# VITA-Group/MM3DGS-SLAM

Measured on AMD Instinct MI355X. Metric: SLAM frames/sec (track+map), TUM fr1/desk-shaped 640x480, higher is better.
Workload: dtype f32

## Files before the change

mm3dgs_slam_amd/csrc/api.hip:

```cpp
#include <math.h>
#include <stdarg.h>
#include <stdio.h>
#include <string.h>
#include "mm3dgs_common.h"
#include <algorithm>
#include "fused_api.h"

static thread_local char g_err[512] = "";
static int fail(int code, const char* fmt, ...) {
  va_list ap;
  va_start(ap, fmt);
  vsnprintf(g_err, sizeof(g_err), fmt, ap);
  va_end(ap);
  return code;
}
static int check_launch(const char* what) {
  hipError_t e = hipGetLastError();
  if (e != hipSuccess) return fail(-10, "%s: %s", what, hipGetErrorString(e));
  return 0;
}

#include <mutex>
#include <vector>
struct KernelProfile {
  std::vector<std::pair<hipEvent_t, hipEvent_t>> pending, pool;
  unsigned long long launches = 0;
  double total_ms = 0.0;
};
static KernelProfile g_prof[MM3DGS_PROF_KERNELS];
static std::mutex g_prof_mu;
static int g_prof_on = 0;
struct ProfScope {
  int k; hipStream_t s; hipEvent_t e1 = nullptr; bool on;
  ProfScope(int k_, hipStream_t s_) : k(k_), s(s_), on(g_prof_on == 1 || (g_prof_on == 2 && (k_ == MM3DGS_PROF_COMPOSITE_BWD || k_ == MM3DGS_PROF_COMPOSITE_BWD_TRACK ||
                                                                                     k_ == MM3DGS_PROF_COMPOSITE_FWD || k_ == MM3DGS_PROF_TRACK_FWD_BWD))) {
    if (on && g_prof_on == 2) {
      static unsigned long long sample[MM3DGS_PROF_KERNELS] = {};
      on = (sample[k_]++ & 63ull) == 0ull;
    }
    if (!on) return;
    std::lock_guard<std::mutex> lk(g_prof_mu);
    std::pair<hipEvent_t, hipEvent_t> ev;
    if (!g_prof[k].pool.empty()) { ev = g_prof[k].pool.back(); g_prof[k].pool.pop_back(); }
    else { (void)hipEventCreate(&ev.first); (void)hipEventCreate(&ev.second); }
    g_prof[k].pending.push_back(ev);
    e1 = ev.second;
    (void)hipEventRecord(ev.first, s);
  }
  ~ProfScope() { if (on) (void)hipEventRecord(e1, s); }
};

__global__ void profile_null_kernel() {}

extern "C" {

void mm3dgs_profile_enable(int on) { g_prof_on = on; }
double mm3dgs_profile_event_overhead_ms(void* stream) {
  hipStream_t s = (hipStream_t)stream;
  hipEvent_t a, b;
  if (hipEventCreate(&a) != hipSuccess || hipEventCreate(&b) != hipSuccess) return 0.0;
  double t[2] = {0.0, 0.0};
  const int reps = 32;
  for (int n = 1; n <= 2; n++) {
    for (int r = 0; r < reps + 4; r++) {
      (void)hipEventRecord(a, s);
      for (int q = 0; q < n; q++) hipLaunchKernelGGL(profile_null_kernel, dim3(1), dim3(64), 0, s);
      (void)hipEventRecord(b, s);
      (void)hipEventSynchronize(b);
      float ms = 0.f;
      if (r >= 4 && hipEventElapsedTime(&ms, a, b) == hipSuccess) t[n - 1] += ms;
    }
  }
  (void)hipEventDestroy(a); (void)hipEventDestroy(b);
  const double o = (2.0 * t[0] - t[1]) / reps;
  return o > 0.0 ? o : 0.0;
}
int mm3dgs_profile_read(int kernel, uint64_t* launches, double* total_ms) {
  if (kernel < 0 || kernel >= MM3DGS_PROF_KERNELS) return fail(-1, "bad kernel id %d", kernel);
  std::lock_guard<std::mutex> lk(g_prof_mu);
  KernelProfile& p = g_prof[kernel];
  for (auto& ev : p.pending) {
    if (hipEventSynchronize(ev.second) == hipSuccess) {
      float ms = 0.f;
      if (hipEventElapsedTime(&ms, ev.first, ev.second) == hipSuccess) { p.total_ms += ms; p.launches++; }
    }
    p.pool.push_back(ev);
  }
  p.pending.clear();
  if (launches) *launches = p.launches;
  if (total_ms) *total_ms = p.total_ms;
  p.launches = 0; p.total_ms = 0.0;
  return 0;
}

const char* mm3dgs_last_error(void) { return g_err; }
int mm3dgs_version(void) { return MM3DGS_ABI_VERSION; }

size_t mm3dgs_geom_bytes(int P) { return geom_bytes_impl(P > 0 ? P : 1); }
size_t mm3dgs_image_bytes(int H, int W) { return image_bytes_impl(H, W); }
size_t mm3dgs_binning_bytes(size_t N) { return binning_bytes_impl(N); }
size_t mm3dgs_backward_scratch_bytes(int P, size_t N) { return bwd_bytes_impl(P, N); }

static int check_common(const Mm3dgsCamera* cam, int P, int M, int C, const float* shs, const float* colors,
                        const float* scales, const float* rots, const float* cov3d) {
  if (!cam) return fail(-1, "camera is NULL");
  if (cam->image_height <= 0 || cam->image_width <= 0) return fail(-1, "bad image size %dx%d", cam->image_height, cam->image_width);
  if (cam->image_height > 16 * 65535 || cam->image_width > 16 * 65535) return fail(-1, "image too large for 16-bit tile coordinates");
  if (P < 0) return fail(-1, "P < 0");
  if (C < 1 || C > MM3DGS_MAX_CHANNELS) return fail(-1, "C=%d outside 1..%d", C, MM3DGS_MAX_CHANNELS);
  if (P == 0) return 0;
  if (!shs && !colors) return fail(-2, "Please provide excatly one of either SHs or precomputed colors!");
  if (shs) {
    if (C < 3) return fail(-2, "SH colour needs C >= 3");
    if (C > 3 && !colors) return fail(-2, "C=%d with SHs needs %d extra precomputed channels", C, C - 3);
    if (cam->sh_degree < 0 || cam->sh_degree > 3) return fail(-2, "sh_degree %d outside 0..3", cam->sh_degree);
    if (M < (cam->sh_degree + 1) * (cam->sh_degree + 1)) return fail(-2, "M=%d too small for sh_degree %d", M, cam->sh_degree);
  }
  if ((scales == nullptr || rots == nullptr) == (cov3d == nullptr))
    return fail(-2, "Please provide exactly one of either scale/rotation pair or precomputed 3D covariance!");
  if (!cam->bg || !cam->viewmatrix || !cam->projmatrix || !cam->campos) return fail(-1, "camera device pointers missing");
  return 0;
}

int mm3dgs_forward_geom(const Mm3dgsCamera* cam, int P, int M, int C, const float* means3D, const float* shs,
                        const float* colors_precomp, const float* opacities, const float* scales,
                        const float* rotations, const float* cov3D_precomp, int32_t* radii, void* geom_state,
                        void* image_state, uint32_t* host_num_rendered, void* stream) {
  int rc = check_common(cam, P, M, C, shs, colors_precomp, scales, rotations, cov3D_precomp);
  if (rc) return rc;
  if (!geom_state || !image_state || (P > 0 && (!means3D || !opacities || !radii))) return fail(-1, "NULL buffer");
  hipStream_t s = (hipStream_t)stream;
  CamDev cd = cam_dev(cam);
  GeomView g = geom_view(geom_state, P > 0 ? P : 1);
  ImageView iv = image_view(image_state, cd.H, cd.W);
  if (hipMemsetAsync(image_state, 0, iv.zero_bytes, s) != hipSuccess) return fail(-10, "memset failed");
  { ProfScope ps(MM3DGS_PROF_PREPROCESS_FWD, s);
    launch_preprocess_fwd(cd, P, M, C, means3D, shs, colors_precomp, opacities, scales, rotations, cov3D_precomp, radii, g, iv, s); }
  { ProfScope ps(MM3DGS_PROF_SCAN, s); launch_scan_tiles(cd.gx * cd.gy, P, g, iv, s); }
  if (host_num_rendered)
    if (hipMemcpyAsync(host_num_rendered, &iv.hdr->num_rendered, sizeof(uint32_t), hipMemcpyDeviceToHost, s) != hipSuccess)
      return fail(-10, "num_rendered copy failed");
  return check_launch("forward_geom");
}

int mm3dgs_forward_raster(const Mm3dgsCamera* cam, int P, int C, const void* geom_state, void* image_state,
                          void* binning_state, size_t N_capacity, float* out_color, void* stream) {
  if (!cam || !geom_state || !image_state || !binning_state || !out_color) return fail(-1, "NULL buffer");
  if (C < 1 || C > MM3DGS_MAX_CHANNELS) return fail(-1, "C=%d outside 1..%d", C, MM3DGS_MAX_CHANNELS);
  hipStream_t s = (hipStream_t)stream;
  CamDev cd = cam_dev(cam);
  GeomView g = geom_view((void*)geom_state, P > 0 ? P : 1);
  ImageView iv = image_view(image_state, cd.H, cd.W);
  BinView b = bin_view(binning_state, N_capacity);
  { ProfScope ps(MM3DGS_PROF_BIN_SORT, s); launch_scatter_sort(cd, P, g, iv, b, N_capacity, nullptr, s); }
  { ProfScope ps(MM3DGS_PROF_COMPOSITE_FWD, s); launch_composite_fwd(cd, C, g, iv, b, N_capacity, out_color, s); }
  return check_launch("forward_raster");
}

int mm3dgs_forward(const Mm3dgsCamera* cam, int P, int M, int C, const float* means3D, const float* shs,
                   const float* colors_precomp, const float* opacities, const float* scales,
                   const float* rotations, const float* cov3D_precomp, float* out_color, int32_t* radii,
                   void* geom_state, void* image_state, void* binning_state, size_t N_capacity, void* stream) {
  int rc = mm3dgs_forward_geom(cam, P, M, C, means3D, shs, colors_precomp, opacities, scales, rotations, cov3D_precomp,
                               radii, geom_state, image_state, nullptr, stream);
  if (rc) return rc;
  return mm3dgs_forward_raster(cam, P, C, geom_state, image_state, binning_state, N_capacity, out_color, stream);
}

int mm3dgs_backward(const Mm3dgsCamera* cam, int P, int M, int C, const float* means3D, const float* shs,
                    const float* colors_precomp, const float* opacities, const float* scales,
                    const float* rotations, const float* cov3D_precomp, const int32_t* radii,
                    const void* geom_state, const void* image_state, const void* binning_state,
                    size_t N_capacity, const float* dL_dout, void* backward_scratch, float* dL_dmeans3D,
                    float* dL_dmeans2D, float* dL_dshs, float* dL_dcolors_precomp, float* dL_dopacities,
                    float* dL_dscales, float* dL_drotations, float* dL_dcov3D, float* dL_dview, float* dL_dproj,
                    float* dL_dcampos, int flags, void* stream) {
  int rc = check_common(cam, P, M, C, shs, colors_precomp, scales, rotations, cov3D_precomp);
  if (rc) return rc;
  if (!geom_state || !image_state || !binning_state || !dL_dout || !backward_scratch || (P > 0 && !radii))
    return fail(-1, "NULL buffer");
  hipStream_t s = (hipStream_t)stream;
  CamDev cd = cam_dev(cam);
  GeomView g = geom_view((void*)geom_state, P > 0 ? P : 1);
  ImageView iv = image_view((void*)image_state, cd.H, cd.W);
  BinView b = bin_view((void*)binning_state, N_capacity);
  BwdView bw = bwd_view(backward_scratch, P, N_capacity);
  { ProfScope ps(MM3DGS_PROF_COMPOSITE_BWD, s); launch_composite_bwd(cd, C, g, iv, b, N_capacity, dL_dout, bw.dsub, s); }
  ProfScope ps_pb(MM3DGS_PROF_PREPROCESS_BWD, s);
  bool want_cam = dL_dview || dL_dproj || dL_dcampos;
  launch_preprocess_bwd(cd, P, M, C, means3D, shs, colors_precomp, opacities, scales, rotations, cov3D_precomp, radii, g, b,
                        N_capacity, bw, dL_dmeans3D, dL_dmeans2D, dL_dshs, dL_dcolors_precomp, dL_dopacities, dL_dscales, dL_drotations,
                        dL_dcov3D, want_cam, flags, s);
  if (want_cam) launch_camgrad_finish(bw, dL_dview, dL_dproj, dL_dcampos, s);
  return check_launch("backward");
}

static void warn_env_once() {
  static const bool done = [] {
    static const char* const names[] = {"MM3DGS_NO_DIRECT_BINS", "MM3DGS_NO_FUSED_SORT", "MM3DGS_NO_FUSED_SCAN", "MM3DGS_NO_FUSED_TRACK", "MM3DGS_NO_FOLDED_LOSS",
                                        "MM3DGS_NO_FORWARD_ROWS", "MM3DGS_NO_FUSED_PROJECT", "MM3DGS_NO_TILE_ORDER", "MM3DGS_NO_POSE_CHAIN", "MM3DGS_TILEMAP",
                                        "MM3DGS_DIRECT_MAX_TILES", "MM3DGS_STATS", "MM3DGS_SLAM_LDS_PAD", "MM3DGS_FWD_LDS_PAD", "MM3DGS_BWD_LDS_PAD"};
    for (const char* n : names) {
      const char* v = getenv(n);
      if (v && *v) fprintf(stderr, "mm3dgs: developer switch %s=%s is set in the environment: it changes which kernels run (include/mm3dgs.h, \"Environment\")\n", n, v);
    }
    return true;
  }();
  (void)done;
}

static SlamIn slam_in(const Mm3dgsSlamInputs* in) {
  SlamIn s;
  s.pose = in->pose; s.xyz = in->xyz; s.f_dc = in->f_dc; s.opacity = in->opacity; s.scaling = in->scaling;
  s.rotation = in->rotation; s.isotropic = in->isotropic; s.world = in->world_means;
  s.sh_deg = (in->f_rest && in->sh_degree > 0) ? in->sh_degree : 0;
  s.f_rest = s.sh_deg ? in->f_rest : nullptr; s.n_rest = s.sh_deg ? in->n_rest : 0;
  s.sh_dir = s.sh_deg ? in->sh_dir : 0;
  return s;
}
static int check_slam(const Mm3dgsCamera* cam, int P, const Mm3dgsSlamInputs* in) {
  warn_env_once();
  if (!cam || !in) return fail(-1, "NULL argument");
  if (cam->image_height <= 0 || cam->image_width <= 0) return fail(-1, "bad image size");
  if (P < 0) return fail(-1, "P < 0");
  if (!cam->bg || !cam->projmatrix) return fail(-1, "camera device pointers missing");
  if (!in->pose) return fail(-1, "pose is NULL");
  if (P > 0 && (!in->xyz || !in->f_dc || !in->opacity || !in->scaling || !in->rotation)) return fail(-1, "NULL Gaussian parameter");
  if (in->sh_degree < 0 || in->sh_degree > 3) return fail(-2, "sh_degree %d outside 0..3", in->sh_degree);
  if (in->sh_dir < 0 || in->sh_dir > 2) return fail(-2, "sh_dir %d outside 0..2", in->sh_dir);
  if (in->sh_degree > 0) {
    if (P > 0 && !in->f_rest) return fail(-2, "sh_degree %d needs the f_rest rows", in->sh_degree);
    if (in->n_rest < (in->sh_degree + 1) * (in->sh_degree + 1) - 1 || in->n_rest > 15) return fail(-2, "n_rest = %d does not hold sh_degree %d (or exceeds 15)", in->n_rest, in->sh_degree);
    if (in->world_means && in->sh_dir != 2) return fail(-2, "world_means = 1 needs sh_dir = 2 (direction from the camera centre), got sh_dir = %d", in->sh_dir);
    if (in->sh_dir == 2 && !in->world_means) return fail(-2, "sh_dir = 2 (direction from the camera centre) needs world_means = 1");
  }
  return 0;
}

static bool slam_fused_sort(int flags) {
  static const int no_fused_sort = env_flag("MM3DGS_NO_FUSED_SORT", 0);
  return (flags & MM3DGS_FWD_SHORT_LISTS) && !no_fused_sort;
}

struct DirectBins { bool on; uint32_t bin_cap, rec_cap, trec_cap; int nblocks, slot_bits; };
static DirectBins slam_direct_bins(int flags, const CamDev& cd, int P, size_t N_capacity) {
  static const int no_direct = env_flag("MM3DGS_NO_DIRECT_BINS", 0);
  static const int no_fused_scan = env_flag("MM3DGS_NO_FUSED_SCAN", 0);
  static const int max_tiles = env_flag("MM3DGS_DIRECT_MAX_TILES", 11264);
  DirectBins d;
  const int T = cd.gx * cd.gy;
  d.nblocks = (P + 255) / 256;
  const size_t nb = (size_t)std::max(d.nblocks, 1);
  d.slot_bits = direct_slot_bits(P);
  d.bin_cap = (uint32_t)std::min<size_t>(N_capacity / (size_t)std::max(T, 1), (size_t)((1u << std::max(d.slot_bits, 1)) - 1u));
  d.rec_cap = (uint32_t)std::min<size_t>((size_t)NLIST * N_capacity / nb, 0xffffffffull / nb);
  d.trec_cap = (uint32_t)std::min<size_t>(N_capacity / nb, 0xffffffffull / nb);
  d.on = (flags & MM3DGS_FWD_DIRECT_BINS) && (flags & MM3DGS_FWD_STATE_CLEAN) && slam_fused_sort(flags) && !no_direct && !no_fused_scan &&
         P > 0 && d.slot_bits >= DIRECT_SLOT_BITS_MIN && T <= max_tiles && T <= MAX_LDS_TILES && d.bin_cap >= 32 && d.rec_cap >= 1024 && d.trec_cap >= 256 &&
         N_capacity >= 4 * (size_t)P;
  return d;
}

static bool slam_tile_table(int flags) { return (flags & MM3DGS_FWD_STATE_CLEAN) && !env_flag("MM3DGS_NO_TILE_ORDER", 0); }
static void slam_refresh_tile_order(const Mm3dgsCamera* cam, void* image_state, int flags, void* stream) {
  if (!cam || !image_state || !slam_tile_table(flags) || cam->image_height <= 0 || cam->image_width <= 0) return;
  if (flags & MM3DGS_FWD_KEEP_TILE_ORDER) return;
  const CamDev cd = cam_dev(cam);
  launch_tile_order(cd.gx * cd.gy, cd.H, cd.W, image_view(image_state, cd.H, cd.W), (hipStream_t)stream);
}

static int slam_forward_impl(const Mm3dgsCamera* cam, int P, const Mm3dgsSlamInputs* in, float* out_color, int32_t* radii,
                             void* geom_state, void* image_state, void* binning_state, size_t N_capacity, int flags, void* stream,
                             const TrackLoss* tl, float* track_dsub = nullptr, bool projected = false, bool pose_chain = false) {
  int rc = check_slam(cam, P, in);
  if (rc) return rc;
  if (!out_color || !geom_state || !image_state || !binning_state || (P > 0 && !radii)) return fail(-1, "NULL buffer");
  hipStream_t s = (hipStream_t)stream;
  CamDev cd = cam_dev(cam);
  GeomView g = geom_view(geom_state, P > 0 ? P : 1);
  ImageView iv = image_view(image_state, cd.H, cd.W);
  BinView b = bin_view(binning_state, N_capacity);
  if (!(flags & MM3DGS_FWD_STATE_CLEAN))
    if (hipMemsetAsync(image_state, 0, iv.zero_bytes, s) != hipSuccess) return fail(-10, "memset failed");
  cd.sort_single = (flags & MM3DGS_FWD_SHORT_LISTS) ? 1 : 0;
  cd.bg_extras = 1;
  cd.state_clean = (flags & MM3DGS_FWD_STATE_CLEAN) ? 1 : 0;
  cd.tile_table = slam_tile_table(flags) ? 1 : 0;
  cd.fused_scan = ((flags & MM3DGS_FWD_STATE_CLEAN) && P > 0 && cd.gx * cd.gy <= MAX_FUSED_SCAN_TILES && !env_flag("MM3DGS_NO_FUSED_SCAN", 0)) ? 1 : 0;
  const bool fused_sort = slam_fused_sort(flags);
  if (tl && !fused_sort) return fail(-1, "internal: folded tracking loss needs the fused sort path");
  const DirectBins db = slam_direct_bins(flags, cd, P, N_capacity);
  cd.trec_cap = db.on ? db.trec_cap : 0u;
  if (db.on) {
    if (!projected) { ProfScope ps(MM3DGS_PROF_PREPROCESS_FWD, s); launch_slam_project_bin(cd, P, slam_in(in), radii, g, iv, b, db.bin_cap, db.rec_cap, db.slot_bits, s, pose_chain); }
    { ProfScope ps(track_dsub ? MM3DGS_PROF_TRACK_FWD_BWD : MM3DGS_PROF_COMPOSITE_FWD, s);
      if (track_dsub) launch_sort_composite_fwd_bwd_track(cd, g, iv, b, N_capacity, out_color, 1, s, *tl, db.nblocks, track_dsub, db.bin_cap, db.slot_bits, pose_chain);
      else launch_sort_composite_fwd6(cd, g, iv, b, N_capacity, out_color, 1, s, tl, db.nblocks, db.bin_cap, db.slot_bits); }
    return check_launch("slam_forward");
  }
  { ProfScope ps(MM3DGS_PROF_PREPROCESS_FWD, s); launch_slam_preprocess_fwd(cd, P, slam_in(in), radii, g, iv, s, nullptr, false, pose_chain); }
  if (!cd.fused_scan) { ProfScope ps(MM3DGS_PROF_SCAN, s); launch_scan_tiles(cd.gx * cd.gy, P, g, iv, s, (flags & MM3DGS_FWD_STATE_CLEAN) ? 1 : 0); }
  { ProfScope ps(MM3DGS_PROF_BIN_SORT, s); launch_scatter_sort(cd, P, g, iv, b, N_capacity, nullptr, s, fused_sort); }
  { ProfScope ps((fused_sort && track_dsub) ? MM3DGS_PROF_TRACK_FWD_BWD : MM3DGS_PROF_COMPOSITE_FWD, s);
    if (fused_sort && track_dsub) launch_sort_composite_fwd_bwd_track(cd, g, iv, b, N_capacity, out_color, (cd.fused_scan || cd.state_clean) ? 1 : 0, s, *tl, 0, track_dsub, 0, DIRECT_SLOT_BITS_MAX, pose_chain);
    else if (fused_sort) launch_sort_composite_fwd6(cd, g, iv, b, N_capacity, out_color, (cd.fused_scan || cd.state_clean) ? 1 : 0, s, tl);
    else launch_composite_fwd(cd, 6, g, iv, b, N_capacity, out_color, s); }
  return check_launch("slam_forward");
}

int mm3dgs_slam_visibility(const Mm3dgsCamera* cam, int P, const Mm3dgsSlamInputs* in, int32_t* radii, uint32_t* seen_count, void* geom_state,
                           void* stream) {
  int rc = check_slam(cam, P, in);
  if (rc) return rc;
  if (!geom_state || (P > 0 && !radii)) return fail(-1, "NULL buffer");
  CamDev cd = cam_dev(cam);
  GeomView g = geom_view(geom_state, P > 0 ? P : 1);
  ImageView iv = {};
  launch_slam_preprocess_fwd(cd, P, slam_in(in), radii, g, iv, (hipStream_t)stream, seen_count, true);
  return check_launch("slam_visibility");
}

int mm3dgs_slam_forward(const Mm3dgsCamera* cam, int P, const Mm3dgsSlamInputs* in, float* out_color, int32_t* radii,
                        void* geom_state, void* image_state, void* binning_state, size_t N_capacity, int flags, void* stream) {
  return slam_forward_impl(cam, P, in, out_color, radii, geom_state, image_state, binning_state, N_capacity, flags, stream, nullptr, nullptr,
                           (flags & MM3DGS_FWD_PROJECTED) != 0);
}

static int map_adam_dev(const Mm3dgsMapAdam* map_adam, MapAdam& ma) {
  if (map_adam->step < 1) return fail(-1, "map Adam step must be >= 1");
  for (int i = 0; i < 5; i++) {
    if (!map_adam->param[i] || !map_adam->exp_avg[i] || !map_adam->exp_avg_sq[i]) return fail(-2, "map Adam group %d has a NULL pointer", i);
    ma.p[i] = map_adam->param[i]; ma.m[i] = map_adam->exp_avg[i]; ma.v[i] = map_adam->exp_avg_sq[i];
    ma.step_size[i] = (float)(map_adam->lr[i] / (1.0 - pow(map_adam->beta1, (double)map_adam->step)));
  }
  ma.omb1 = (float)(1.0 - map_adam->beta1); ma.beta2 = (float)map_adam->beta2; ma.omb2 = (float)(1.0 - map_adam->beta2);
  ma.eps = (float)map_adam->eps;
  ma.bc2s = (float)sqrt(1.0 - pow(map_adam->beta2, (double)map_adam->step));
  ma.opt_mask = map_adam->opt_mask;
  ma.rp = map_adam->rest_param; ma.rm = map_adam->rest_exp_avg; ma.rv = map_adam->rest_exp_avg_sq;
  if (ma.rp && (!ma.rm || !ma.rv)) return fail(-2, "map Adam: the f_rest group has a NULL moment pointer");
  ma.rest_step_size = (float)(map_adam->rest_lr / (1.0 - pow(map_adam->beta1, (double)map_adam->step)));
  ma.on = 1;
  return 0;
}

static int slam_backward_impl(const Mm3dgsCamera* cam, int P, const Mm3dgsSlamInputs* in, const int32_t* radii,
                              const void* geom_state, const void* image_state, const void* binning_state, size_t N_capacity,
                              const float* dL_dout, void* backward_scratch, const Mm3dgsSlamGrads* grads, float* dL_dpose,
                              const Mm3dgsPoseAdam* pose_adam, const Mm3dgsMapAdam* map_adam, int flags, void* stream, const TrackLoss* tl,
                              float* prior_loss4 = nullptr, int dl_planes = 6, bool compositor_done = false, const float* fuse_next_pose = nullptr,
                              bool* fused_out = nullptr, bool pose_chain = false) {
  PoseLossScale pls = {nullptr, 0, 0.f, nullptr};
  if (tl && tl->defer_scale) { pls.rows = tl->partial; pls.nrows = ((tl->cfg.W + 15) / 16) * ((tl->cfg.H + 15) / 16); pls.w_l1 = tl->cfg.w_l1; pls.loss4 = tl->loss4; }
  int rc = check_slam(cam, P, in);
  if (rc) return rc;
  if (!geom_state || !image_state || !binning_state || !dL_dout || !backward_scratch || (P > 0 && !radii)) return fail(-1, "NULL buffer");
  hipStream_t s = (hipStream_t)stream;
  CamDev cd = cam_dev(cam);
  GeomView g = geom_view((void*)geom_state, P > 0 ? P : 1);
  ImageView iv = image_view((void*)image_state, cd.H, cd.W);
  BinView b = bin_view((void*)binning_state, N_capacity);
  BwdView bw = bwd_view(backward_scratch, P, N_capacity);
  cd.bg_extras = 1;
  cd.tile_table = slam_tile_table(flags) ? 1 : 0;
  const DirectBins db_bwd = slam_direct_bins(flags, cd, P, N_capacity);
  cd.trec_cap = db_bwd.on ? db_bwd.trec_cap : 0u;
  SlamGrads sg = {};
  if (grads) {
    const bool any = grads->d_xyz || grads->d_f_dc || grads->d_opacity || grads->d_scaling || grads->d_rotation;
    const bool all = grads->d_xyz && grads->d_f_dc && grads->d_opacity && grads->d_scaling && grads->d_rotation;
    if (any && !all) return fail(-2, "Gaussian gradient outputs must be all set or all NULL");
    if (grads->max_radii2D && (!grads->grad_accum || !grads->denom)) return fail(-2, "statistics outputs must be all set or all NULL");
    sg.d_xyz = grads->d_xyz; sg.d_f_dc = grads->d_f_dc; sg.d_opacity = grads->d_opacity; sg.d_scaling = grads->d_scaling;
    sg.d_rotation = grads->d_rotation; sg.max_radii2D = grads->max_radii2D; sg.grad_accum = grads->grad_accum; sg.denom = grads->denom;
    sg.d_f_rest = (all && in->sh_degree > 0) ? grads->d_f_rest : nullptr;
    if (all && in->sh_degree > 0 && !grads->d_f_rest) return fail(-2, "sh_degree > 0: the gradient outputs need d_f_rest too");
  }
  PoseAdam pa = {};
  if (pose_adam && pose_adam->pose) {
    if (!pose_adam->m || !pose_adam->v || !pose_adam->step) return fail(-2, "pose Adam state missing");
    pa.pose = pose_adam->pose; pa.m = pose_adam->m; pa.v = pose_adam->v; pa.step = pose_adam->step;
    pa.lr_q = pose_adam->lr_q; pa.lr_t = pose_adam->lr_t; pa.beta1 = pose_adam->beta1; pa.beta2 = pose_adam->beta2; pa.eps = (float)pose_adam->eps;
    if (pose_adam->prior_pose && (pose_adam->prior_w_t != 0.f || pose_adam->prior_w_q != 0.f)) {
      pa.prior = pose_adam->prior_pose; pa.prior_w_t = pose_adam->prior_w_t; pa.prior_w_q = pose_adam->prior_w_q;
    }
    pa.best = pose_adam->best;
  }
  MapAdam ma;
  memset(&ma, 0, sizeof(ma));
  if (map_adam)
    if (int rc2 = map_adam_dev(map_adam, ma)) return rc2;
  const bool sh = in->sh_degree > 0 && in->f_rest;
  if (sh && ma.on && !ma.rp) return fail(-2, "sh_degree > 0: the map Adam state needs the f_rest group");
  const bool tracking = sg.d_xyz == nullptr && !ma.on && !sh;
  if (tl && !tracking && !tl->dmaps) return fail(-1, "internal: a loss folded into the mapping backward needs the SSIM maps");
  if (pose_chain && !tracking) return fail(-1, "internal: the pose chain is a tracking-mode path");
  if (!compositor_done)
  { ProfScope ps(tracking ? MM3DGS_PROF_COMPOSITE_BWD_TRACK : MM3DGS_PROF_COMPOSITE_BWD, s);
    launch_composite_bwd_slam(cd, tracking, g, iv, b, N_capacity, dL_dout, bw.dsub, s, tl, dl_planes, pose_chain); }
  if (pose_chain) {
    ProfScope ps(MM3DGS_PROF_PREPROCESS_BWD, s);
    launch_slam_pose_finish(bw.dsub, cd.gx * cd.gy, in->pose, dL_dpose, pa, s, pls.rows ? &pls : nullptr, prior_loss4, &iv.hdr->overflow);
    return check_launch("slam_backward");
  }
  const bool fuse = fuse_next_pose && !tracking && ma.on && db_bwd.on && !dL_dpose && !pa.pose && !sg.d_xyz && !sh;
  if (fused_out) *fused_out = fuse;
  if (fuse) {
    ProfScope ps(MM3DGS_PROF_PREPROCESS_BWD, s);
    launch_slam_bwd_project(cd, P, slam_in(in), (int32_t*)radii, g, image_view((void*)image_state, cd.H, cd.W), b, N_capacity, bw, sg, ma, fuse_next_pose,
                            db_bwd.bin_cap, db_bwd.rec_cap, db_bwd.slot_bits, s);
  } else
  { ProfScope ps(MM3DGS_PROF_PREPROCESS_BWD, s); launch_slam_preprocess_bwd(cd, P, slam_in(in), radii, g, b, N_capacity, bw, sg, dL_dpose, pa, ma, s, pls.rows ? &pls : nullptr, prior_loss4, db_bwd.on, &iv.hdr->overflow); }
  return check_launch("slam_backward");
}

int mm3dgs_slam_backward(const Mm3dgsCamera* cam, int P, const Mm3dgsSlamInputs* in, const int32_t* radii,
                         const void* geom_state, const void* image_state, const void* binning_state, size_t N_capacity,
                         const float* dL_dout, void* backward_scratch, const Mm3dgsSlamGrads* grads, float* dL_dpose,
                         const Mm3dgsPoseAdam* pose_adam, const Mm3dgsMapAdam* map_adam, int flags, void* stream) {
  return slam_backward_impl(cam, P, in, radii, geom_state, image_state, binning_state, N_capacity, dL_dout, backward_scratch, grads, dL_dpose,
                            pose_adam, map_adam, flags, stream, nullptr);
}

static size_t loss_rows(int H, int W) { return (size_t)((W + 15) / 16) * ((H + 15) / 16); }
static LossCfg loss_cfg_dev(const Mm3dgsLossConfig* c) {
  LossCfg lc;
  lc.H = c->H; lc.W = c->W; lc.w_l1 = c->w_l1; lc.w_ssim = c->w_ssim; lc.w_pearson = c->w_pearson; lc.l1_mask = c->l1_mask;
  lc.pearson_mask = c->pearson_mask; lc.pearson_invert = c->pearson_invert; lc.sil_thr = c->sil_thr;
  for (int i = 0; i < 11; i++) lc.window[i] = c->window[i];
  lc.w_depth = c->w_depth_l1; lc.depth_mask = c->depth_l1_mask; lc.l1_sum = c->l1_sum;
  return lc;
}
static bool loss_is_variant(const Mm3dgsLossConfig* c) { return c->w_depth_l1 != 0.f || c->l1_sum != 0 || (c->l1_mask & 2) != 0; }
static int loss_cfg_check(const Mm3dgsLossConfig* c, const float* ref) {
  if (c->w_pearson != 0.f && !ref) return fail(-2, "Pearson term needs a reference depth");
  if ((c->w_depth_l1 != 0.f || (c->l1_mask & 2)) && !ref) return fail(-2, "depth-L1 term / { ref > 0 } mask needs a reference depth");
  if (c->w_depth_l1 != 0.f && c->w_pearson != 0.f) return fail(-2, "the depth-L1 and Pearson terms are exclusive");
  return 0;
}
size_t mm3dgs_loss_work_bytes(int H, int W) {
  return 256 + align_up((size_t)9 * H * W * 4, 256) + align_up(loss_rows(H, W) * 12 * 8, 256);
}

int mm3dgs_loss(const Mm3dgsLossConfig* c, const float* out6, const float* gt_color, const float* ref, void* work, float* dL,
                float* loss4, void* stream) {
  if (!c || !out6 || !gt_color || !work || !dL) return fail(-1, "NULL argument");
  if (c->H <= 0 || c->W <= 0) return fail(-1, "bad image size");
  if ((double)c->H * c->W * 36.0 >= 4294967296.0) return fail(-1, "image too large for the loss kernels' 32-bit offsets");
  if (int rc = loss_cfg_check(c, ref)) return rc;
  LossCfg lc = loss_cfg_dev(c);
  hipStream_t s = (hipStream_t)stream;
  ProfScope ps(MM3DGS_PROF_LOSS, s);
  char* w = (char*)work;
  launch_loss(lc, out6, gt_color, ref, (float*)(w + 256), (double*)w, (double*)(w + 256 + align_up((size_t)9 * c->H * c->W * 4, 256)), dL,
              loss4, s);
  return check_launch("loss");
}

int mm3dgs_slam_track(int n_iter, const Mm3dgsCamera* cam, int P, const Mm3dgsSlamInputs* in, float* out_color, int32_t* radii,
                      void* geom_state, void* image_state, void* binning_state, size_t N_capacity, int fwd_flags,
                      const Mm3dgsLossConfig* loss_cfg, const float* gt_color, const float* ref, void* loss_work, float* dL_dout,
                      float* loss4, void* backward_scratch, const Mm3dgsPoseAdam* pose_adam, void* stream) {
  if (n_iter < 0) return fail(-1, "n_iter < 0");
  if (!pose_adam || !pose_adam->pose) return fail(-2, "tracking needs the pose Adam state");
  Mm3dgsSlamGrads none;
  memset(&none, 0, sizeof(none));
  if (!loss_cfg || !gt_color || !loss_work || !dL_dout) return fail(-1, "NULL argument");
  if (int rc = loss_cfg_check(loss_cfg, ref)) return rc;
  const int no_fold = env_flag("MM3DGS_NO_FOLDED_LOSS", 0);
  const bool sh = in->sh_degree > 0 && in->f_rest;
  const bool fold = !no_fold && !sh && !loss_is_variant(loss_cfg) && loss_cfg->w_ssim == 0.f && slam_fused_sort(fwd_flags) && cam->image_height > 0 && cam->image_width > 0;
  TrackLoss tl = {};
  if (fold) {
    tl.cfg = loss_cfg_dev(loss_cfg);
    char* w = (char*)loss_work;
    tl.gt = gt_color; tl.ref = ref; tl.out = out_color; tl.sums = (const double*)w;
    tl.partial = (double*)(w + 256 + align_up((size_t)9 * loss_cfg->H * loss_cfg->W * 4, 256));
    tl.loss4 = loss4;
    tl.defer_scale = loss_cfg->w_pearson == 0.f ? 1 : 0;
    if (loss_cfg->H != cam->image_height || loss_cfg->W != cam->image_width) return fail(-1, "loss and camera image sizes differ");
  }
  const bool fuse_track = fold && tl.defer_scale && !env_flag("MM3DGS_NO_FUSED_TRACK", 0) && backward_scratch;
  float* track_dsub = nullptr;
  if (fuse_track) {
    track_dsub = bwd_view(backward_scratch, P, N_capacity).dsub;
  }
  const bool pose_chain = !in->world_means && !sh && backward_scratch && !env_flag("MM3DGS_NO_POSE_CHAIN", 0) &&
                          bwd_bytes_impl(P, N_capacity) >= (size_t)tiles_x(cam->image_width) * tiles_y(cam->image_height) * 32 * sizeof(float);
  if (n_iter > 0) slam_refresh_tile_order(cam, image_state, fwd_flags, stream);
  for (int it = 0; it < n_iter; it++) {
    int rc = slam_forward_impl(cam, P, in, out_color, radii, geom_state, image_state, binning_state, N_capacity, fwd_flags, stream, fold ? &tl : nullptr, track_dsub, false, pose_chain);
    if (rc) return rc;
    if (fold) {
      if (!tl.defer_scale) {
        ProfScope ps(MM3DGS_PROF_LOSS, (hipStream_t)stream);
        launch_loss_finish(tl.cfg, (double*)loss_work, tl.partial, (hipStream_t)stream);
      }
    } else {
      rc = mm3dgs_loss(loss_cfg, out_color, gt_color, ref, loss_work, dL_dout, loss4, stream);
      if (rc) return rc;
    }
    rc = slam_backward_impl(cam, P, in, radii, geom_state, image_state, binning_state, N_capacity, dL_dout, backward_scratch, &none,
                            nullptr, pose_adam, nullptr, fwd_flags, stream, fold ? &tl : nullptr, loss4, 6, fuse_track, nullptr, nullptr, pose_chain);
    if (rc) return rc;
  }
  return 0;
}

int mm3dgs_slam_map(int n_iter, const Mm3dgsMapView* views, const Mm3dgsCamera* cam, int P, const Mm3dgsSlamInputs* in, float* out_color,
                    int32_t* radii, void* geom_state, void* image_state, void* binning_state, size_t N_capacity, int fwd_flags,
                    const Mm3dgsLossConfig* loss_cfg, void* loss_work, float* dL_dout, float* loss4, void* backward_scratch,
                    const Mm3dgsSlamGrads* grads_stats, const Mm3dgsMapAdam* map_adam, void* stream) {
  if (n_iter < 0) return fail(-1, "n_iter < 0");
  if (n_iter > 0 && (!views || !in)) return fail(-1, "NULL argument");
  if (n_iter > 0 && !map_adam && !(grads_stats && grads_stats->d_xyz)) return fail(-1, "neither an Adam state nor gradient outputs");
  Mm3dgsSlamGrads sg;
  memset(&sg, 0, sizeof(sg));
  if (grads_stats) sg = *grads_stats;
  Mm3dgsMapAdam ad;
  memset(&ad, 0, sizeof(ad));
  if (map_adam) ad = *map_adam;
  Mm3dgsSlamInputs si = *in;
  if (n_iter > 0 && (!loss_cfg || !loss_work || !dL_dout)) return fail(-1, "NULL argument");
  const int no_rows = env_flag("MM3DGS_NO_FORWARD_ROWS", 0);
  const bool rows = n_iter > 0 && !no_rows && !loss_is_variant(loss_cfg) && loss_cfg->w_ssim != 0.f && slam_fused_sort(fwd_flags) && loss_cfg->H == cam->image_height &&
                    loss_cfg->W == cam->image_width;
  TrackLoss tl = {};
  LossCfg lc = {};
  char* w = (char*)loss_work;
  double* sums = (double*)w;
  float* dmaps = (float*)(w + 256);
  double* partial = n_iter > 0 ? (double*)(w + 256 + align_up((size_t)9 * loss_cfg->H * loss_cfg->W * 4, 256)) : nullptr;
  if (rows) {
    lc = loss_cfg_dev(loss_cfg);
    tl.cfg = lc; tl.out = out_color; tl.sums = sums; tl.partial = partial; tl.loss4 = nullptr; tl.defer_scale = 0;
  }
  const int no_fuse_proj = env_flag("MM3DGS_NO_FUSED_PROJECT", 0);
  bool projected = (fwd_flags & MM3DGS_FWD_PROJECTED) != 0;
  if (n_iter > 0) slam_refresh_tile_order(cam, image_state, fwd_flags, stream);
  for (int it = 0; it < n_iter; it++) {
    if (!views[it].pose || !views[it].gt_color) return fail(-1, "view %d: NULL pose or colour target", it);
    if (loss_cfg->w_pearson != 0.f && !views[it].ref_depth_or_null) return fail(-2, "view %d: Pearson term needs a reference depth", it);
    if ((loss_cfg->w_depth_l1 != 0.f || (loss_cfg->l1_mask & 2)) && !views[it].ref_depth_or_null) return fail(-2, "view %d: depth-L1 term needs a reference depth", it);
    si.pose = views[it].pose;
    int rc;
    if (rows) {
      tl.gt = views[it].gt_color; tl.ref = views[it].ref_depth_or_null;
      rc = slam_forward_impl(cam, P, &si, out_color, radii, geom_state, image_state, binning_state, N_capacity, fwd_flags, stream, &tl, nullptr, projected);
      if (rc) return rc;
      const bool fold_grad = !env_flag("MM3DGS_NO_FOLDED_LOSS", 0);
      { ProfScope ps(MM3DGS_PROF_LOSS, (hipStream_t)stream);
        launch_loss_after_forward_rows(lc, out_color, tl.gt, tl.ref, dmaps, sums, partial, fold_grad ? nullptr : dL_dout, (hipStream_t)stream); }
      if (loss4 && it == n_iter - 1) launch_loss_finish(lc, sums, partial, (hipStream_t)stream, loss4);
      rc = check_launch("loss");
      if (rc) return rc;
      tl.dmaps = fold_grad ? dmaps : nullptr;
      if (views[it].pose_adam_or_null && views[it].dpose_out_or_null) return fail(-2, "view %d: either a pose step or a pose-gradient output", it);
      const float* next_pose = (!no_fuse_proj && map_adam && it + 1 < n_iter && !views[it].pose_adam_or_null && !views[it + 1].pose_adam_or_null &&
                                !views[it].dpose_out_or_null && views[it + 1].pose) ? views[it + 1].pose : nullptr;
      projected = false;
      rc = slam_backward_impl(cam, P, &si, radii, geom_state, image_state, binning_state, N_capacity, dL_dout, backward_scratch, &sg, views[it].dpose_out_or_null,
                              views[it].pose_adam_or_null, map_adam ? &ad : nullptr, fwd_flags, stream, fold_grad ? &tl : nullptr, nullptr, 4, false,
                              next_pose, &projected);
    } else {
      rc = mm3dgs_slam_forward(cam, P, &si, out_color, radii, geom_state, image_state, binning_state, N_capacity,
                               it == 0 ? fwd_flags : (fwd_flags & ~MM3DGS_FWD_PROJECTED), stream);
      if (rc) return rc;
      rc = mm3dgs_loss(loss_cfg, out_color, views[it].gt_color, views[it].ref_depth_or_null, loss_work, dL_dout, loss4, stream);
      if (rc) return rc;
      rc = mm3dgs_slam_backward(cam, P, &si, radii, geom_state, image_state, binning_state, N_capacity, dL_dout, backward_scratch, &sg,
                                views[it].dpose_out_or_null, views[it].pose_adam_or_null, map_adam ? &ad : nullptr, fwd_flags, stream);
    }
    if (rc) return rc;
    ad.step++;
  }
  return 0;
}

int mm3dgs_adam(const Mm3dgsAdamGroup* groups, int n_groups, int step, double beta1, double beta2, double eps, void* stream) {
  if (!groups || n_groups < 0 || n_groups > 8) return fail(-1, "bad group table");
  if (step < 1) return fail(-1, "step must be >= 1");
  AdamArgs a;
  a.ngroups = n_groups; a.omb1 = (float)(1.0 - beta1); a.beta2 = (float)beta2; a.omb2 = (float)(1.0 - beta2); a.eps = (float)eps;
  const double bc1 = 1.0 - pow(beta1, (double)step);
  a.bc2s = (float)sqrt(1.0 - pow(beta2, (double)step));
  for (int i = 0; i < n_groups; i++) {
    if (groups[i].n && (!groups[i].param || !groups[i].grad || !groups[i].exp_avg || !groups[i].exp_avg_sq)) return fail(-1, "NULL in group %d", i);
    a.grp[i].p = groups[i].param; a.grp[i].g = groups[i].grad; a.grp[i].m = groups[i].exp_avg; a.grp[i].v = groups[i].exp_avg_sq;
    a.grp[i].n = groups[i].n; a.grp[i].step_size = (float)(groups[i].lr / bc1);
  }
  hipStream_t s = (hipStream_t)stream;
  ProfScope ps(MM3DGS_PROF_ADAM, s);
  launch_fused_adam(a, s);
  return check_launch("adam");
}

int mm3dgs_slam_direct_bins(const Mm3dgsCamera* cam, int P, size_t N_capacity, int fwd_flags) {
  if (!cam || P <= 0 || cam->image_height <= 0 || cam->image_width <= 0) return 0;
  return slam_direct_bins(fwd_flags, cam_dev(cam), P, N_capacity).on ? 1 : 0;
}

int mm3dgs_slam_adam_project(const Mm3dgsCamera* cam, int P, const Mm3dgsSlamInputs* in, const Mm3dgsSlamGrads* grads, const Mm3dgsMapAdam* adam,
                             int32_t* radii, void* geom_state, void* image_state, void* binning_state, size_t N_capacity, int fwd_flags, void* stream) {
  int rc = check_slam(cam, P, in);
  if (rc) return rc;
  if (!grads || !adam || !geom_state || !image_state || !binning_state || (P > 0 && !radii)) return fail(-1, "NULL argument");
  if (!grads->d_xyz || !grads->d_f_dc || !grads->d_opacity || !grads->d_scaling || !grads->d_rotation) return fail(-2, "all five gradient arrays are needed");
  if (in->sh_degree > 0 && !grads->d_f_rest) return fail(-2, "sh_degree %d needs grads->d_f_rest", in->sh_degree);
  if (in->sh_degree > 0 && (!adam->rest_param || !adam->rest_exp_avg || !adam->rest_exp_avg_sq))
    return fail(-2, "sh_degree %d needs the f_rest group of the map Adam (rest_param / rest_exp_avg / rest_exp_avg_sq)", in->sh_degree);
  hipStream_t s = (hipStream_t)stream;
  CamDev cd = cam_dev(cam);
  cd.bg_extras = 1;
  cd.tile_table = slam_tile_table(fwd_flags) ? 1 : 0;
  const DirectBins db = slam_direct_bins(fwd_flags, cd, P, N_capacity);
  if (!db.on) return fail(-3, "mm3dgs_slam_adam_project needs direct bins (flags / map size / capacity)");
  cd.trec_cap = db.trec_cap;
  MapAdam ma;
  memset(&ma, 0, sizeof(ma));
  if ((rc = map_adam_dev(adam, ma))) return rc;
  SlamGrads sg = {};
  sg.d_xyz = grads->d_xyz; sg.d_f_dc = grads->d_f_dc; sg.d_opacity = grads->d_opacity; sg.d_scaling = grads->d_scaling; sg.d_rotation = grads->d_rotation;
  sg.d_f_rest = in->sh_degree > 0 ? grads->d_f_rest : nullptr;
  { ProfScope ps(MM3DGS_PROF_ADAM, s);
    launch_slam_adam_project(cd, P, slam_in(in), radii, geom_view(geom_state, P > 0 ? P : 1), image_view(image_state, cd.H, cd.W), bin_view(binning_state, N_capacity),
                             sg, ma, in->pose, db.bin_cap, db.rec_cap, db.slot_bits, s); }
  return check_launch("slam_adam_project");
}

int mm3dgs_covisibility_ratio(int H, int W, const float* depth, const float* silhouette, const float* keyframe_pose, const float* current_pose,
                              float fx, float fy, float cx, float cy, uint32_t* counts, void* stream) {
  if (H < 0 || W < 0 || !depth || !silhouette || !keyframe_pose || !current_pose || !counts) return fail(-1, "covisibility_ratio: bad argument");
  launch_covisibility_ratio(H, W, depth, silhouette, keyframe_pose, current_pose, fx, fy, cx, cy, counts, (hipStream_t)stream);
  return check_launch("covisibility_ratio");
}

int mm3dgs_propagate_const_vel(const float* pose_m1, const float* pose_m2, float* out_pose, void* stream) {
  if (!pose_m1 || !pose_m2 || !out_pose) return fail(-1, "propagate_const_vel: NULL argument");
  launch_propagate_const_vel(pose_m1, pose_m2, out_pose, (hipStream_t)stream);
  return check_launch("propagate_const_vel");
}

int mm3dgs_propagate_imu(const float* pose_m1, const float* pose_m2, const float* imu6, int n, const float* c2i, double dt_cam, double dt_imu,
                         double gx, double gy, double gz, float* out_pose, void* stream) {
  if (!pose_m1 || !pose_m2 || !c2i || !out_pose) return fail(-1, "propagate_imu: NULL argument");
  if (n < 0) return fail(-2, "propagate_imu: n = %d < 0", n);
  if (n > 0 && !imu6) return fail(-1, "propagate_imu: imu6 is NULL with n = %d samples", n);
  if (!isfinite(dt_cam) || !isfinite(dt_imu) || dt_cam == 0.0) return fail(-2, "propagate_imu: dt_cam = %g (finite, not 0) / dt_imu = %g (finite)", dt_cam, dt_imu);
  if (!isfinite(gx) || !isfinite(gy) || !isfinite(gz)) return fail(-2, "propagate_imu: gravity (%g, %g, %g) is not finite", gx, gy, gz);
  launch_propagate_imu(pose_m1, pose_m2, imu6, n, c2i, dt_cam, dt_imu, gx, gy, gz, out_pose, (hipStream_t)stream);
  return check_launch("propagate_imu");
}

int mm3dgs_prune_mask(int P, const float* opacity, const float* log_scales, const float* max_radii2D, float min_opacity, float max_scale,
                      float max_screen_size, uint8_t* keep, uint32_t* n_pruned_accum, void* stream) {
  if (P < 0) return fail(-1, "P < 0");
  if (P > 0 && (!opacity || !log_scales || !keep || !n_pruned_accum)) return fail(-1, "NULL argument");
  launch_prune_mask(P, opacity, log_scales, max_radii2D, min_opacity, max_scale, max_screen_size, max_radii2D ? 1 : 0, keep, n_pruned_accum,
                    (hipStream_t)stream);
  return check_launch("prune_mask");
}
size_t mm3dgs_compact_work_bytes(size_t n) { return align_up(((n + 255) / 256 + 1) * 4, 256); }
int mm3dgs_compact_plan(size_t n, const uint8_t* keep, void* work, uint32_t* n_keep, void* stream) {
  if (n > 0x7fffffffull) return fail(-1, "n too large");
  if (!work || !n_keep || (n > 0 && !keep)) return fail(-1, "NULL argument");
  launch_compact_plan((int)n, keep, (uint32_t*)work, n_keep, (hipStream_t)stream);
  return check_launch("compact_plan");
}
int mm3dgs_compact_rows(size_t n, const uint8_t* keep, const void* work, const Mm3dgsCompactArray* arrays, int n_arrays, void* stream) {
  if (n > 0x7fffffffull) return fail(-1, "n too large");
  if (n_arrays < 0 || n_arrays > 32) return fail(-1, "at most 32 arrays per call");
  if (n > 0 && (!keep || !work || (n_arrays > 0 && !arrays))) return fail(-1, "NULL argument");
  CompactTable t;
  t.n_arrays = 0;
  for (int a = 0; a < n_arrays; a++) {
    if (arrays[a].width < 0) return fail(-1, "array %d: negative width", a);
    if (arrays[a].width == 0) continue;
    if (!arrays[a].src || !arrays[a].dst) return fail(-1, "array %d: NULL pointer", a);
    t.src[t.n_arrays] = arrays[a].src; t.dst[t.n_arrays] = arrays[a].dst; t.width[t.n_arrays] = arrays[a].width; t.n_arrays++;
  }
  launch_compact_rows((int)n, keep, (const uint32_t*)work, t, (hipStream_t)stream);
  return check_launch("compact_rows");
}
int mm3dgs_seed_gaussians(int H, int W, const float* color, const float* depth, const uint8_t* keep, const void* work, const float* pose, float fx,
                          float fy, float cx, float cy, uint32_t row0, const Mm3dgsSeedOutputs* out, int n_rest, void* stream) {
  if (H <= 0 || W <= 0 || (double)H * W > 2147483647.0) return fail(-1, "bad image size");
  if (!color || !depth || !keep || !work || !pose || !out) return fail(-1, "NULL argument");
  if (!out->xyz || !out->f_dc || !out->opacity || !out->scaling || !out->rotation || !out->rgb || (n_rest > 0 && !out->f_rest))
    return fail(-1, "NULL output array");
  SeedOut o = {out->xyz, out->f_dc, out->f_rest, out->opacity, out->scaling, out->rotation, out->rgb, n_rest > 0 ? n_rest : 0};
  launch_seed_gaussians(H, W, color, depth, keep, (const uint32_t*)work, pose, fx, fy, cx, cy, row0, o, (hipStream_t)stream);
  return check_launch("seed_gaussians");
}

static size_t densify_cls_bytes(size_t P) { return align_up(P, 256); }
size_t mm3dgs_densify_work_bytes(size_t P) { return densify_cls_bytes(P) + align_up((3 * ((P + 255) / 256) + 1) * 4, 256); }
int mm3dgs_densify_plan(size_t P, const float* grad_accum, const float* denom, const float* log_scales, float max_grad, float max_clone_scale,
                        void* work, uint32_t* counts, void* stream) {
  if (P > 0x7fffffffull) return fail(-1, "P too large");
  if (!work || !counts || (P > 0 && (!grad_accum || !denom || !log_scales))) return fail(-1, "NULL argument");
  launch_densify_plan((int)P, grad_accum, denom, log_scales, max_grad, max_clone_scale, (uint8_t*)work,
                      (uint32_t*)((char*)work + densify_cls_bytes(P)), counts, (hipStream_t)stream);
  return check_launch("densify_plan");
}
int mm3dgs_densify_rows(size_t P, const void* work, uint32_t n_keep, uint32_t n_clone, uint32_t n_split, int N, uint32_t seed,
                        const Mm3dgsDensifyState* st, void* stream) {
  if (P > 0x7fffffffull) return fail(-1, "P too large");
  if (N < 1 || N > 64) return fail(-1, "N out of range");
  if ((uint64_t)n_keep + n_split != P || n_clone > n_keep) return fail(-1, "counts do not describe a plan of %zu rows", P);
  if ((uint64_t)n_keep + n_clone + (uint64_t)N * n_split > 0x7fffffffull) return fail(-1, "densified map too large");
  if (P == 0) return 0;
  if (!work || !st || !st->grad_accum || !st->denom || !st->max_radii2D) return fail(-1, "NULL argument");
  DensifyTable t = {};
  for (int a = 0; a < 7; a++) {
    const Mm3dgsDensifyGroup& g = st->group[a];
    if (g.width < 0) return fail(-1, "group %d: negative width", a);
    if (g.width > 0 && (!g.src || !g.dst)) return fail(-1, "group %d: NULL pointer", a);
    if ((g.m_dst && !g.m_src) || (g.v_dst && !g.v_src)) return fail(-1, "group %d: moment destination without source", a);
    t.src[a] = g.src; t.dst[a] = g.dst; t.m_src[a] = g.m_src; t.m_dst[a] = g.m_dst; t.v_src[a] = g.v_src; t.v_dst[a] = g.v_dst; t.width[a] = g.width;
  }
  if (n_split > 0 && (t.width[0] != 3 || t.width[4] != 3 || t.width[5] != 4)) return fail(-1, "split needs xyz[3], scaling[3], rotation[4]");
  t.grad_accum = st->grad_accum; t.denom = st->denom; t.max_radii2D = st->max_radii2D; t.parent = st->parent;
  launch_densify_rows((int)P, (const uint8_t*)work, (const uint32_t*)((const char*)work + densify_cls_bytes(P)), n_keep, n_clone, n_split, N, seed,
                      (float)(0.8 * (double)N), t, (hipStream_t)stream);
  return check_launch("densify_rows");
}

int mm3dgs_mark_visible(const Mm3dgsCamera* cam, int P, const float* means3D, uint8_t* visible, void* stream) {
  if (!cam || !cam->viewmatrix || (P > 0 && (!means3D || !visible))) return fail(-1, "NULL buffer");
  launch_mark_visible(cam_dev(cam), P, means3D, visible, (hipStream_t)stream);
  return check_launch("mark_visible");
}

}
```

mm3dgs_slam_amd/csrc/fused.hip:

```cpp
#pragma clang fp contract(on)
#include "mm3dgs_math.h"
#include "fused_api.h"
#include "composite_common.h"
#include "tile_mask.h"

#define FB 256
#define SLAM_BWD_FB 256
#define SH_C0F 0.28209479177387814f

struct PoseDev { float R[3][3]; float t[3]; float qn[4]; float inv_norm; };

__device__ __forceinline__ PoseDev load_pose(const float* __restrict__ pose) {
  PoseDev p;
  float w = pose[0], x = pose[1], y = pose[2], z = pose[3];
  float n = sqrtf(w * w + x * x + y * y + z * z);
  p.inv_norm = 1.f / n;
  p.qn[0] = w * p.inv_norm; p.qn[1] = x * p.inv_norm; p.qn[2] = y * p.inv_norm; p.qn[3] = z * p.inv_norm;
  quat_to_R(p.qn, p.R);
  p.t[0] = pose[4]; p.t[1] = pose[5]; p.t[2] = pose[6];
  return p;
}

__device__ __forceinline__ void slam_cov3d_vals(const float q[4], const float ls[3], bool isotropic, float mod, float S3[3][3],
                                                float R[3][3], float sm[3], float qn[4], float& qinv) {
  float n = sqrtf(q[0] * q[0] + q[1] * q[1] + q[2] * q[2] + q[3] * q[3]);
  n = fmaxf(n, 1e-12f);
  qinv = 1.f / n;
  qn[0] = q[0] * qinv; qn[1] = q[1] * qinv; qn[2] = q[2] * qinv; qn[3] = q[3] * qinv;
  quat_to_R(qn, R);
  sm[0] = mod * expf(ls[0]);
  sm[1] = isotropic ? sm[0] : mod * expf(ls[1]);
  sm[2] = isotropic ? sm[0] : mod * expf(ls[2]);
  float Mx[3][3];
#pragma unroll
  for (int i = 0; i < 3; i++)
#pragma unroll
    for (int k = 0; k < 3; k++) Mx[i][k] = R[i][k] * sm[k];
#pragma unroll
  for (int i = 0; i < 3; i++)
#pragma unroll
    for (int j = 0; j < 3; j++) S3[i][j] = Mx[i][0] * Mx[j][0] + Mx[i][1] * Mx[j][1] + Mx[i][2] * Mx[j][2];
}

__device__ __forceinline__ void slam_cov3d(const SlamIn& in, int idx, float mod, float S3[3][3], float R[3][3], float sm[3],
                                           float qn[4], float& qinv) {
  const float* qp = in.rotation + (size_t)idx * 4;
  const float* lp = in.scaling + (size_t)idx * 3;
  const float q[4] = {qp[0], qp[1], qp[2], qp[3]}, ls[3] = {lp[0], lp[1], lp[2]};
  slam_cov3d_vals(q, ls, in.isotropic != 0, mod, S3, R, sm, qn, qinv);
}

struct Projected { uint32_t r0, r1; float4 sA, sB; BlkRect br; float z; int32_t rad; uint32_t cl; };
struct RawGaussian { float x[3], q[4], ls[3], fd[3], op; };

__device__ __forceinline__ void pose_view_matrix(const PoseDev& ps, float V[16]) {
#pragma unroll
  for (int i = 0; i < 3; i++) {
#pragma unroll
    for (int j = 0; j < 3; j++) V[i * 4 + j] = ps.R[j][i];
    V[i * 4 + 3] = 0.f;
    V[12 + i] = ps.t[i];
  }
  V[15] = 1.f;
}
__device__ __forceinline__ void pose_chain_record(const CamDev& cam, const float* __restrict__ PV, const float p[3], const float x[3], const Ewa& e,
                                                  const float S3[3][3], float qa, float qb, float qc, float pw, float hx, float hy,
                                                  float* __restrict__ rec) {
  float Kq[3][3];
#pragma unroll
  for (int col = 0; col < 3; col++) {
    const float gA = col == 0 ? -0.5f : 0.f, gB = col == 1 ? -1.f : 0.f, gC = col == 2 ? -0.5f : 0.f;
    float GA[2][3], dA[2][3], dm[3];
    cov2d_grad_to_dA(e, S3, conic_grad_to_cov2d(e.a, e.b, e.c, gA, gB, gC), GA, dA);
    dJ_to_dmean(cam, e, dA[0][0], dA[0][2], dA[1][1], dA[1][2], dm);
    Kq[0][col] = dm[0]; Kq[1][col] = dm[1]; Kq[2][col] = dm[2];
  }
  float Jp[3][2];
  const float sx = 0.5f * cam.W, sy = 0.5f * cam.H;
#pragma unroll
  for (int i = 0; i < 3; i++) {
    Jp[i][0] = PV[i * 4 + 0] * (sx * pw) - PV[i * 4 + 3] * (sx * hx * pw * pw);
    Jp[i][1] = PV[i * 4 + 1] * (sy * pw) - PV[i * 4 + 3] * (sy * hy * pw * pw);
  }
  float4* o = (float4*)rec;
  float Kp[3][2];
#pragma unroll
  for (int i = 0; i < 3; i++) {
    Kp[i][0] = -(Jp[i][0] * qa + Jp[i][1] * qb);
    Kp[i][1] = -(Jp[i][0] * qb + Jp[i][1] * qc);
  }
  o[0] = make_float4(Kp[0][0], Kp[0][1], Kp[1][0], Kp[1][1]);
  o[1] = make_float4(Kp[2][0], Kp[2][1], Kq[0][0], Kq[0][1]);
  o[2] = make_float4(Kq[0][2], Kq[1][0], Kq[1][1], Kq[1][2]);
  o[3] = make_float4(Kq[2][0], Kq[2][1], Kq[2][2], x[0]);
  o[4] = make_float4(x[1], x[2], 0.f, 0.f);
}

template <int SHDIR>
__device__ __forceinline__ void sh_dir_vec(const PoseDev& ps, const float x[3], const float p[3], float v[3]) {
  static_assert(SHDIR >= 0 && SHDIR <= 2, "sh_dir is 0, 1 or 2");
#pragma unroll
  for (int j = 0; j < 3; j++) {
    if constexpr (SHDIR == 0) v[j] = p[j];
    else if constexpr (SHDIR == 1) v[j] = x[j];
    else v[j] = x[j] + ps.R[0][j] * ps.t[0] + ps.R[1][j] * ps.t[1] + ps.R[2][j] * ps.t[2];
  }
}

template <bool SH = false, int SHDIR = 0>
__device__ __forceinline__ Projected slam_project_vals(const CamDev& cam, bool live, int idx, const float* __restrict__ pose, bool isotropic,
                                                       const RawGaussian& rg, int32_t* __restrict__ radii, const GeomView& g, bool world = false,
                                                       bool want_poserec = false, const float* __restrict__ rest = nullptr, int sh_deg = 0) {
  const float* PV = cam.proj;
  const float Vi[16] = {1.f, 0.f, 0.f, 0.f, 0.f, 1.f, 0.f, 0.f, 0.f, 0.f, 1.f, 0.f, 0.f, 0.f, 0.f, 1.f};
  const PoseDev ps = load_pose(pose);
  float p[3] = {0.f, 0.f, 0.f};
  const float* q_raw = rg.q; const float* ls_raw = rg.ls; const float* fd_raw = rg.fd;
  const float op_raw = rg.op;
  if (live) {
#pragma unroll
    for (int i = 0; i < 3; i++) p[i] = ps.R[i][0] * rg.x[0] + ps.R[i][1] * rg.x[1] + ps.R[i][2] * rg.x[2] + ps.t[i];
  }
  Projected o;
  o.r0 = 0; o.r1 = 0; o.rad = 0; o.z = 0.f; o.cl = 0;
  o.sA = make_float4(0.f, 0.f, 0.f, 0.f); o.sB = o.sA;
  o.br.bx0 = 0; o.br.by0 = 0; o.br.bw = 0; o.br.bh = 0;
  if (live && p[2] > 0.2f) {
    const HomPoint h = hom_project(PV, p);
    float S3[3][3], R[3][3], sm[3], qn[4], qinv;
    slam_cov3d_vals(q_raw, ls_raw, isotropic, cam.scale_modifier, S3, R, sm, qn, qinv);
    Ewa e;
    if (world) {
      float V[16];
      pose_view_matrix(ps, V);
      ewa_project(cam, V, rg.x, S3, e);
    } else {
      ewa_project(cam, Vi, p, S3, e);
    }
    float det = e.a * e.c - e.b * e.b;
    float px = ((h.hx * h.pw + 1.f) * cam.W - 1.f) * 0.5f;
    float py = ((h.hy * h.pw + 1.f) * cam.H - 1.f) * 0.5f;
    if (det != 0.f && isfinite(px) && isfinite(py)) {
      float dinv = 1.f / det;
      float mid = 0.5f * (e.a + e.c);
      float lam = mid + sqrtf(fmaxf(0.1f, mid * mid - det));
      float rf = ceilf(3.f * sqrtf(lam));
      float gxf = (float)cam.gx + 1.f, gyf = (float)cam.gy + 1.f;
      int minx = min(cam.gx, max(0, (int)fminf(fmaxf((px - rf) / TILE, -1.f), gxf)));
      int miny = min(cam.gy, max(0, (int)fminf(fmaxf((py - rf) / TILE, -1.f), gyf)));
      int maxx = min(cam.gx, max(0, (int)fminf(fmaxf((px + rf + (TILE - 1)) / TILE, -1.f), gxf)));
      int maxy = min(cam.gy, max(0, (int)fminf(fmaxf((py + rf + (TILE - 1)) / TILE, -1.f), gyf)));
      if ((maxx - minx) * (maxy - miny) > 0) {
        o.rad = (int32_t)fminf(rf, 2.0e9f);
        o.r0 = (uint32_t)minx | ((uint32_t)miny << 16);
        o.r1 = (uint32_t)maxx | ((uint32_t)maxy << 16);
        const float* fd = fd_raw;
        float c0 = SH_C0F * fd[0] + 0.5f, c1 = SH_C0F * fd[1] + 0.5f, c2 = SH_C0F * fd[2] + 0.5f;
        if constexpr (SH) {
          float v[3];
          sh_dir_vec<SHDIR>(ps, rg.x, p, v);
          const float inv = 1.f / sqrtf(v[0] * v[0] + v[1] * v[1] + v[2] * v[2]);
          float bb[16];
          sh_basis(sh_deg, v[0] * inv, v[1] * inv, v[2] * inv, bb);
          const int nb = (sh_deg + 1) * (sh_deg + 1);
          c0 = bb[0] * fd[0]; c1 = bb[0] * fd[1]; c2 = bb[0] * fd[2];
#pragma unroll
          for (int k = 1; k < 16; k++)
            if (k < nb) { c0 += bb[k] * rest[(k - 1) * 3]; c1 += bb[k] * rest[(k - 1) * 3 + 1]; c2 += bb[k] * rest[(k - 1) * 3 + 2]; }
          c0 += 0.5f; c1 += 0.5f; c2 += 0.5f;
        }
        o.cl = (c0 < 0.f ? 1u : 0u) | (c1 < 0.f ? 2u : 0u) | (c2 < 0.f ? 4u : 0u);
        g.clamped[idx] = (uint8_t)o.cl;
        const float z = p[2];
        const float zc = world ? ps.R[0][2] * rg.x[0] + ps.R[1][2] * rg.x[1] + ps.R[2][2] * rg.x[2] : p[2];
        const float op = 1.f / (1.f + expf(-op_raw));
        float4* sp = (float4*)(g.splat + (size_t)idx * SPLAT_F);
        o.sA = make_float4(px, py, e.c * dinv, -e.b * dinv); o.sB = make_float4(e.a * dinv, op, fmaxf(c0, 0.f), fmaxf(c1, 0.f));
        sp[0] = o.sA;
        sp[1] = o.sB;
        o.br = block_rect(o.sA, o.sB, o.r0, o.r1);
        sp[2] = make_float4(fmaxf(c2, 0.f), zc, 1.f, zc * zc);
        g.depth[idx] = z;
        o.z = z;
        if (want_poserec && !world)
          pose_chain_record(cam, PV, p, rg.x, e, S3, e.c * dinv, -e.b * dinv, e.a * dinv, h.pw, h.hx, h.hy, g.poserec + (size_t)idx * POSEREC_F);
      }
    }
  }
  if (live) {
    radii[idx] = o.rad;
    g.rect[(size_t)idx * 2] = o.r0;
    g.rect[(size_t)idx * 2 + 1] = o.r1;
  }
  return o;
}

template <bool SH = false, int SHDIR = 0>
__device__ __forceinline__ Projected slam_project_one(const CamDev& cam, int P, int idx, const SlamIn& in, int32_t* __restrict__ radii,
                                                      const GeomView& g, bool want_poserec = false) {
  const bool live = idx < P;
  RawGaussian rg = {{0.f, 0.f, 0.f}, {1.f, 0.f, 0.f, 0.f}, {0.f, 0.f, 0.f}, {0.f, 0.f, 0.f}, 0.f};
  if (live) {
#pragma unroll
    for (int k = 0; k < 3; k++) rg.x[k] = in.xyz[(size_t)idx * 3 + k];
#pragma unroll
    for (int k = 0; k < 4; k++) rg.q[k] = in.rotation[(size_t)idx * 4 + k];
#pragma unroll
    for (int k = 0; k < 3; k++) { rg.ls[k] = in.scaling[(size_t)idx * 3 + k]; rg.fd[k] = in.f_dc[(size_t)idx * 3 + k]; }
    rg.op = in.opacity[idx];
  }
  return slam_project_vals<SH, SHDIR>(cam, live, idx, in.pose, in.isotropic != 0, rg, radii, g, in.world != 0, want_poserec,
                               SH ? in.f_rest + (size_t)(live ? idx : 0) * (size_t)in.n_rest * 3 : nullptr, in.sh_deg);
}

template <bool SH, int SHDIR = 0>
__global__ void __launch_bounds__(FB)
slam_preprocess_fwd_kernel(CamDev cam, int P, SlamIn in, int32_t* __restrict__ radii, GeomView g, ImageView iv, int lds_tiles,
                           int vis_only, uint32_t* __restrict__ seen, int want_poserec) {
  extern __shared__ uint32_t hist[];
  const int T = cam.gx * cam.gy;
  for (int t = threadIdx.x; t < lds_tiles; t += FB) hist[t] = 0;
  if (lds_tiles) __syncthreads();
  const int idx = blockIdx.x * FB + threadIdx.x;
  const bool live = idx < P;
  const Projected pr = slam_project_one<SH, SHDIR>(cam, P, idx, in, radii, g, want_poserec != 0);
  const uint32_t r0 = pr.r0, r1 = pr.r1;
  const int32_t rad = pr.rad;
  if (vis_only) {
    if (live && seen && rad > 0) seen[idx] += 1u;
    return;
  }
  {
    const int minx = r0 & 0xffff, miny = r0 >> 16, maxx = r1 & 0xffff, maxy = r1 >> 16;
    const int w = maxx - minx, area = w * (maxy - miny);
    {
      __shared__ uint32_t wtot[FB / 64];
      const int ln = threadIdx.x & 63, wvi = threadIdx.x >> 6;
      const uint32_t x = wave_scan_incl((uint32_t)area);
      if (ln == 63) wtot[wvi] = x;
      __syncthreads();
      uint32_t pre = 0;
      for (int q = 0; q < wvi; q++) pre += wtot[q];
      if (live) g.tileoff[idx] = pre + x - (uint32_t)area;
      if (threadIdx.x == FB - 1) g.block_tiles[blockIdx.x] = pre + x;
    }
    uint32_t* cnt = lds_tiles ? hist : iv.tile_count;
    const int lane = threadIdx.x & 63;
    unsigned long long big = __ballot(area > 32);
    if (area > 0 && area <= 32)
      for (int y = miny; y < maxy; y++)
        for (int x = minx; x < maxx; x++) atomicAdd(&cnt[y * cam.gx + x], 1u);
    while (big) {
      const int src = __ffsll((long long)big) - 1;
      big &= big - 1;
      const int sminx = __builtin_amdgcn_readlane(minx, src), sminy = __builtin_amdgcn_readlane(miny, src);
      const int sw = __builtin_amdgcn_readlane(w, src), sarea = __builtin_amdgcn_readlane(area, src);
      for (int k = lane; k < sarea; k += 64) atomicAdd(&cnt[(sminy + k / sw) * cam.gx + sminx + k % sw], 1u);
    }
  }
  if (lds_tiles) {
    __syncthreads();
    for (int t = threadIdx.x; t < T; t += FB) {
      uint32_t c = hist[t];
      if (c) atomicAdd(&iv.tile_count[t], c);
    }
  }
}

#define SLAM_PICK_SH(K, in) ((in).sh_deg <= 0 ? K<false, 0> : (in).sh_dir == 2 ? K<true, 2> : (in).sh_dir == 1 ? K<true, 1> : K<true, 0>)

void launch_slam_preprocess_fwd(const CamDev& cam, int P, const SlamIn& in, int32_t* radii, GeomView g, ImageView iv, hipStream_t s,
                                uint32_t* seen, bool visibility_only, bool want_poserec) {
  if (P <= 0) return;
  const int T = cam.gx * cam.gy;
  const int lds_tiles = (T <= MAX_LDS_TILES && !visibility_only) ? T : 0;
  hipLaunchKernelGGL(SLAM_PICK_SH(slam_preprocess_fwd_kernel, in), dim3((P + FB - 1) / FB), dim3(FB), (size_t)lds_tiles * 4, s, cam, P, in, radii, g, iv,
                     lds_tiles, visibility_only ? 1 : 0, seen, want_poserec && in.sh_deg <= 0 ? 1 : 0);
}

struct PairCtx {
  MaskConsts mc; BlkRect br; uint32_t khi, idbits; int minx, miny, w, area;
  uint32_t trec0;
};
__device__ __forceinline__ uint32_t emit_pair(const PairCtx& c, int k, int ttx, int tty, uint32_t* hist, int gx, uint32_t cap, const BinView& b,
                                              bool have_mask = false, uint32_t mask_in = 0u) {
  const int t = tty * gx + ttx;
  const uint32_t slot = atomicAdd(&hist[t], 1u);
  uint32_t mask = 0;
  if (slot < cap) {
    mask = have_mask ? mask_in : tile_block_mask_in_rect(c.mc, ttx, tty, c.br);
    const size_t at = (size_t)t * cap + slot;
    b.keys[at] = ((unsigned long long)c.khi << 32) | (unsigned long long)(c.idbits | slot);
    b.payload[at] = (unsigned long long)mask | ((unsigned long long)(c.trec0 == 0xffffffffu ? 0xffffffffu : c.trec0 + (uint32_t)k) << 32);
  }
  return mask;
}

__device__ __forceinline__ void slam_bin_pairs(const CamDev& cam, int P, int idx, const Projected& pr, const GeomView& g, const ImageView& iv,
                                               const BinView& b, uint32_t cap, uint32_t rec_cap, int slot_bits, uint32_t* hist) {
  const int T = cam.gx * cam.gy;
  const int tid = threadIdx.x, lane = tid & 63, wvi = tid >> 6;
  const bool live = idx < P;
  PairCtx c;
  c.mc = mask_consts(pr.sA, pr.sB);
  c.br = pr.br;
  c.minx = pr.r0 & 0xffff; c.miny = pr.r0 >> 16;
  c.w = (int)(pr.r1 & 0xffff) - c.minx;
  c.area = c.w * ((int)(pr.r1 >> 16) - c.miny);
  c.khi = __float_as_uint(pr.z);
  c.idbits = (uint32_t)idx << slot_bits;
  {
    __shared__ uint32_t wtot2[FB / 64];
    const uint32_t x2 = wave_scan_incl((uint32_t)c.area);
    if (lane == 63) wtot2[wvi] = x2;
    __syncthreads();
    uint32_t pre2 = 0;
    for (int q = 0; q < wvi; q++) pre2 += wtot2[q];
    const uint32_t plocal = pre2 + x2 - (uint32_t)c.area;
    if (live) g.tileoff[idx] = plocal;
    c.trec0 = plocal + (uint32_t)c.area <= cam.trec_cap ? (uint32_t)blockIdx.x * cam.trec_cap + plocal : 0xffffffffu;
    if (tid == FB - 1) {
      g.block_tiles[blockIdx.x] = pre2 + x2;
      if (pre2 + x2 > cam.trec_cap) iv.hdr->overflow = 1u;
    }
  }
  constexpr int OWN = 4;
  unsigned long long big = __ballot(c.area > 32);
  unsigned long long m64 = 0ull;
  uint32_t empty4 = 0u;
  const bool droppable = c.area > 0 && c.area <= 32;
  if (droppable) {
    int ttx = c.minx, tty = c.miny;
    const int kmax = PROBE(cam, 7) ? min(c.area, OWN) : c.area;
    for (int k = 0; k < kmax; k++) {
      bool count = true;
      if (k < OWN) {
        const uint32_t mk = tile_block_mask_in_rect(c.mc, ttx, tty, c.br);
        m64 |= (unsigned long long)mk << (16 * k);
        count = mk != 0u;
        empty4 |= count ? 0u : (1u << k);
      }
      if (count) atomicAdd(&hist[tty * cam.gx + ttx], 1u);
      if (++ttx == c.minx + c.w) { ttx = c.minx; tty++; }
    }
  }
  if (live) g.clamped[idx] = (uint8_t)(pr.cl | (empty4 << 4));
  if (PROBE(cam, 8)) big = 0ull;
  for (unsigned long long bb = big; bb; bb &= bb - 1) {
    const int src = __ffsll((long long)bb) - 1;
    const int sminx = __builtin_amdgcn_readlane(c.minx, src), sminy = __builtin_amdgcn_readlane(c.miny, src);
    const int sw = __builtin_amdgcn_readlane(c.w, src), sarea = __builtin_amdgcn_readlane(c.area, src);
    for (int k = lane; k < sarea; k += 64) atomicAdd(&hist[(sminy + k / sw) * cam.gx + sminx + k % sw], 1u);
  }
  __syncthreads();
  for (int t = tid; t < T; t += FB) {
    const uint32_t n = hist[t];
    if (n) hist[t] = atomicAdd(&iv.cursor[t], n);
  }
  __syncthreads();
  {
    int ttx = c.minx, tty = c.miny;
    for (int k = 0; k < min(c.area, OWN); k++) {
      if (!((empty4 >> k) & 1u)) emit_pair(c, k, ttx, tty, hist, cam.gx, cap, b, droppable, (uint32_t)(m64 >> (16 * k)) & 0xffffu);
      if (++ttx == c.minx + c.w) { ttx = c.minx; tty++; }
    }
  }
  const uint32_t incl = wave_scan_incl((uint32_t)max(c.area - OWN, 0));
  const uint32_t S = PROBE(cam, 6) ? 0u : (uint32_t)__builtin_amdgcn_readlane((int)incl, 63);
  if (S) {
    __shared__ uint32_t s_pref[FB / 64][64];
    __shared__ PairCtx s_ctx[FB / 64][64];
    s_pref[wvi][lane] = incl;
    s_ctx[wvi][lane] = c;
    __builtin_amdgcn_wave_barrier();
    for (uint32_t i = (uint32_t)lane; i < S; i += 64u) {
      int lo = 0, hi = 63;
#pragma unroll
      for (int st = 0; st < 6; st++) {
        const int mid = (lo + hi) >> 1;
        if (s_pref[wvi][mid] > i) hi = mid; else lo = mid + 1;
      }
      const int o = min(lo, 63);
      const uint32_t excl = o ? s_pref[wvi][o - 1] : 0u;
      const PairCtx oc = s_ctx[wvi][o];
      const int k = OWN + (int)(i - excl);
      emit_pair(oc, k, oc.minx + k % oc.w, oc.miny + k / oc.w, hist, cam.gx, cap, b);
    }
  }
}

__device__ __forceinline__ int slam_bin_prologue(const CamDev& cam, const ImageView& iv, uint32_t cap, uint32_t* hist) {
  const int T = cam.gx * cam.gy;
  const int tid = threadIdx.x;
  for (int t = tid; t < T; t += FB) hist[t] = 0;
  if (blockIdx.x == 0 && tid == 0) iv.hdr->bin_cap = cap;
  return blockIdx.x * FB + tid;
}

template <bool SH, int SHDIR = 0>
__global__ void __launch_bounds__(FB)
slam_project_bin_kernel(CamDev cam, int P, SlamIn in, int32_t* __restrict__ radii, GeomView g, ImageView iv, BinView b, uint32_t cap,
                        uint32_t rec_cap, int slot_bits, int want_poserec) {
  extern __shared__ uint32_t hist[];
  const int idx = slam_bin_prologue(cam, iv, cap, hist);
  const Projected pr = slam_project_one<SH, SHDIR>(cam, P, idx, in, radii, g, want_poserec != 0);
  slam_bin_pairs(cam, P, idx, pr, g, iv, b, cap, rec_cap, slot_bits, hist);
}

void launch_slam_project_bin(const CamDev& cam, int P, const SlamIn& in, int32_t* radii, GeomView g, ImageView iv, BinView b, uint32_t bin_cap,
                             uint32_t rec_cap, int slot_bits, hipStream_t s, bool want_poserec) {
  if (P <= 0) return;
  const int T = cam.gx * cam.gy;
  hipLaunchKernelGGL(SLAM_PICK_SH(slam_project_bin_kernel, in), dim3((P + FB - 1) / FB), dim3(FB), (size_t)T * 4, s, cam, P, in, radii, g, iv, b, bin_cap,
                     rec_cap, slot_bits, want_poserec && in.sh_deg <= 0 ? 1 : 0);
}

template <bool TRACK>
__device__ __forceinline__ void gather_tile_records(int area, uint32_t first, const float* __restrict__ dtile, float4& acc0, float4& acc1, float4& acc2,
                                                    uint32_t skip4) {
  constexpr int RECF = TRACK ? REC_TRACK_F : REC_MAP_F;
  const int lane = threadIdx.x & 63;
  const bool big = area > 16;
  const int n_own = big ? 0 : area;
  for (int k0 = 0; __ballot(k0 < n_own) != 0ull; k0 += 4) {
    float4 a[4], b4[4], c4[4];
    bool on[4];
#pragma unroll
    for (int u = 0; u < 4; u++) {
      on[u] = k0 + u < n_own && !((skip4 >> (k0 + u)) & 1u);
      const float* r = dtile + (on[u] ? (size_t)(first + (uint32_t)(k0 + u)) * RECF : (size_t)0);
      a[u] = ld4u(r); b4[u] = ld4u(r + 4);
      c4[u] = TRACK ? make_float4(0.f, 0.f, 0.f, 0.f) : ld4u(r + 8);
    }
#pragma unroll
    for (int u = 0; u < 4; u++) {
      acc0.x += on[u] ? a[u].x : 0.f; acc0.y += on[u] ? a[u].y : 0.f; acc0.z += on[u] ? a[u].z : 0.f; acc0.w += on[u] ? a[u].w : 0.f;
      acc1.x += on[u] ? b4[u].x : 0.f; acc1.y += on[u] ? b4[u].y : 0.f; acc1.z += on[u] ? b4[u].z : 0.f; acc1.w += on[u] ? b4[u].w : 0.f;
      if (!TRACK) { acc2.x += on[u] ? c4[u].x : 0.f; acc2.y += on[u] ? c4[u].y : 0.f; }
    }
  }
  for (unsigned long long bigs = __ballot(big); bigs; bigs &= bigs - 1ull) {
    const int src = __ffsll((long long)bigs) - 1;
    const int sarea = __builtin_amdgcn_readlane(area, src);
    const uint32_t sfirst = (uint32_t)__builtin_amdgcn_readlane((int)first, src);
    const uint32_t sskip = (uint32_t)__builtin_amdgcn_readlane((int)skip4, src);
    float v[RECF];
#pragma unroll
    for (int f = 0; f < RECF; f++) v[f] = 0.f;
    for (int k = lane; k < sarea; k += 64) {
      if (k < 4 && ((sskip >> k) & 1u)) continue;
      const float* r = dtile + (size_t)(sfirst + (uint32_t)k) * RECF;
#pragma unroll
      for (int f = 0; f < RECF; f++) v[f] += r[f];
    }
#pragma unroll
    for (int f = 0; f < RECF; f++) v[f] = wave_sum(v[f]);
    if (lane == src) {
      acc0 = make_float4(v[0], v[1], v[2], v[3]);
      acc1 = make_float4(v[4], v[5], v[6], TRACK ? 0.f : v[RECF > 7 ? 7 : 0]);
      if (!TRACK) acc2 = make_float4(v[RECF > 8 ? 8 : 0], v[RECF > 9 ? 9 : 0], 0.f, 0.f);
    }
  }
}

#define NPOSE 12
template <bool TRACK, bool DIRECT, bool WORLD = false, bool SH = false, int SHDIR = 0>
__device__ __forceinline__ void slam_bwd_body(const CamDev& cam, int P, const SlamIn& in, const int32_t* __restrict__ radii, const GeomView& g,
                                              uint32_t N_cap, const float* __restrict__ dsub, float* __restrict__ posepartial, const SlamGrads& out,
                                              const MapAdam& ma, RawGaussian* stepped, const uint32_t* __restrict__ ovf) {
  const int idx = blockIdx.x * SLAM_BWD_FB + threadIdx.x;
  const uint32_t ovf_word = ovf != nullptr ? __builtin_nontemporal_load(ovf) : 0u;
  const float* PV = cam.proj;
  const float Vi[16] = {1.f, 0.f, 0.f, 0.f, 0.f, 1.f, 0.f, 0.f, 0.f, 0.f, 1.f, 0.f, 0.f, 0.f, 0.f, 1.f};
  const PoseDev ps = load_pose(in.pose);
  float cg[NPOSE];
#pragma unroll
  for (int k = 0; k < NPOSE; k++) cg[k] = 0.f;
  float4 acc0 = make_float4(0.f, 0.f, 0.f, 0.f), acc1 = acc0, acc2 = acc0;
  int rad = 0;
  uint32_t cl_bits = 0;
  float4 sA = make_float4(0.f, 0.f, 0.f, 0.f), sB = sA;
  float px3[3] = {0.f, 0.f, 0.f}, q_raw[4] = {1.f, 0.f, 0.f, 0.f}, ls_raw[3] = {0.f, 0.f, 0.f}, op_raw = 0.f;
  {
    uint32_t first = 0;
    int area = 0;
    uint32_t r0 = 0, r1 = 0, toff = 0, btile = 0, clb = 0;
    if (idx < P) {
      clb = g.clamped[idx];
#pragma unroll
      for (int k = 0; k < 3; k++) { px3[k] = in.xyz[(size_t)idx * 3 + k]; ls_raw[k] = in.scaling[(size_t)idx * 3 + k]; }
#pragma unroll
      for (int k = 0; k < 4; k++) q_raw[k] = in.rotation[(size_t)idx * 4 + k];
      op_raw = in.opacity[idx];
      rad = radii[idx];
      r0 = g.rect[(size_t)idx * 2]; r1 = g.rect[(size_t)idx * 2 + 1];
      toff = g.tileoff[idx];
      if (!DIRECT) btile = g.block_tiles[idx >> 8];
      const float4* spl = (const float4*)(g.splat + (size_t)idx * SPLAT_F);
      sA = spl[0]; sB = spl[1];
    }
    if (r1 != r0) {
      area = ((int)(r1 & 0xffff) - (int)(r0 & 0xffff)) * ((int)(r1 >> 16) - (int)(r0 >> 16));
      first = DIRECT ? (uint32_t)(idx >> 8) * cam.trec_cap + toff : btile + toff;
      const bool fits = DIRECT ? (toff + (uint32_t)area <= cam.trec_cap) : true;
      if (!fits || (size_t)first + (size_t)area > (size_t)N_cap) area = 0;
    }
    gather_tile_records<TRACK>(area, first, dsub + (size_t)NLIST * (size_t)N_cap * SPLAT_F, acc0, acc1, acc2, DIRECT ? (clb >> 4) : 0u);
    cl_bits = clb;
  }
  const bool skip = ovf_word != 0u;
  if (skip) rad = 0;
  if (idx < P) {
    float dxyz[3] = {0.f, 0.f, 0.f}, dfd[3] = {0.f, 0.f, 0.f}, dls[3] = {0.f, 0.f, 0.f}, dqr[4] = {0.f, 0.f, 0.f, 0.f};
    float dlogit = 0.f, gnorm = 0.f;
    constexpr int AG_OFF[5] = {0, 3, 6, 7, 10}, AG_N[5] = {3, 3, 1, 3, 4};
    float ap[14], am[14], av[14];
    float shb[16], shg[3] = {0.f, 0.f, 0.f};
    float shw[3] = {0.f, 0.f, 0.f};
    if constexpr (SH) {
#pragma unroll
      for (int k = 0; k < 16; k++) shb[k] = 0.f;
    }
    if (ma.on) {
#pragma unroll
      for (int gq = 0; gq < 5; gq++)
#pragma unroll
        for (int c = 0; c < AG_N[gq]; c++) {
          const size_t off = (size_t)idx * AG_N[gq] + c;
          ap[AG_OFF[gq] + c] = ma.p[gq][off]; am[AG_OFF[gq] + c] = ma.m[gq][off]; av[AG_OFF[gq] + c] = ma.v[gq][off];
        }
    }
    if (rad > 0) {
      const float4 sp0 = sA, sp1 = sB;
      const float qa = sp0.z, qb = sp0.w, qc = sp1.x;
      const float M0 = acc0.x, m_x = acc0.y, m_xx = acc0.z;
      const float m_y = TRACK ? acc1.x : acc1.w, m_xy = TRACK ? acc1.y : acc2.x, m_yy = TRACK ? acc1.z : acc2.y;
      const float dc0 = acc0.w, dc1 = acc1.x, dc2 = acc1.y;
      const float dz_tot = TRACK ? acc0.w : acc1.z;
      const float gpx = -(qa * m_x + qb * m_y), gpy = -(qc * m_y + qb * m_x);
      const float gA = -0.5f * m_xx, gB = -m_xy, gC = -0.5f * m_yy;
      const float x0 = px3[0], x1 = px3[1], x2 = px3[2];
      float p[3];
#pragma unroll
      for (int i = 0; i < 3; i++) p[i] = ps.R[i][0] * x0 + ps.R[i][1] * x1 + ps.R[i][2] * x2 + ps.t[i];
      float S3[3][3], R[3][3], sm[3], qn[4], qinv;
      slam_cov3d_vals(q_raw, ls_raw, in.isotropic != 0, cam.scale_modifier, S3, R, sm, qn, qinv);
      Ewa e;
      constexpr bool world = WORLD;
      if (world) {
        float V[16];
        pose_view_matrix(ps, V);
        const float xw[3] = {x0, x1, x2};
        ewa_project(cam, V, xw, S3, e);
      } else {
        ewa_project(cam, Vi, p, S3, e);
      }
      float GA[2][3], dS[3][3], dA[2][3];
      cov2d_grad_to_dA(e, S3, conic_grad_to_cov2d(e.a, e.b, e.c, gA, gB, gC), GA, dA);
#pragma unroll
      for (int i = 0; i < 3; i++)
#pragma unroll
        for (int j = 0; j < 3; j++) dS[i][j] = e.A[0][i] * GA[0][j] + e.A[1][i] * GA[1][j];
      {
        const float s01 = 0.5f * (dS[0][1] + dS[1][0]), s02 = 0.5f * (dS[0][2] + dS[2][0]), s12 = 0.5f * (dS[1][2] + dS[2][1]);
        dS[0][1] = s01; dS[1][0] = s01; dS[0][2] = s02; dS[2][0] = s02; dS[1][2] = s12; dS[2][1] = s12;
      }
      float dJ00 = dA[0][0], dJ02 = dA[0][2], dJ11 = dA[1][1], dJ12 = dA[1][2];
      float dRc[3][3] = {{0.f, 0.f, 0.f}, {0.f, 0.f, 0.f}, {0.f, 0.f, 0.f}};
      if (world) {
        dJ00 = dA[0][0] * ps.R[0][0] + dA[0][1] * ps.R[0][1] + dA[0][2] * ps.R[0][2];
        dJ02 = dA[0][0] * ps.R[2][0] + dA[0][1] * ps.R[2][1] + dA[0][2] * ps.R[2][2];
        dJ11 = dA[1][0] * ps.R[1][0] + dA[1][1] * ps.R[1][1] + dA[1][2] * ps.R[1][2];
        dJ12 = dA[1][0] * ps.R[2][0] + dA[1][1] * ps.R[2][1] + dA[1][2] * ps.R[2][2];
#pragma unroll
        for (int i = 0; i < 3; i++) {
          dRc[0][i] = e.J00 * dA[0][i];
          dRc[1][i] = e.J11 * dA[1][i];
          dRc[2][i] = e.J02 * dA[0][i] + e.J12 * dA[1][i];
        }
      }
      float dm[3];
      dJ_to_dmean(cam, e, dJ00, dJ02, dJ11, dJ12, dm);
      const HomPoint h = hom_project(PV, p);
      const float hx = h.hx, hy = h.hy, pw = h.pw;
      const float gnx = gpx * 0.5f * cam.W, gny = gpy * 0.5f * cam.H;
      gnorm = sqrtf(gnx * gnx + gny * gny);
      const float dhx = gnx * pw, dhy = gny * pw, dhw = -(gnx * hx + gny * hy) * pw * pw;
#pragma unroll
      for (int i = 0; i < 3; i++) dm[i] += PV[i * 4 + 0] * dhx + PV[i * 4 + 1] * dhy + PV[i * 4 + 3] * dhw;
      if (!world) dm[2] += dz_tot;
      if constexpr (SH) {
        static_assert(!TRACK, "the SH path runs on mapping-layout records");
        static_assert(WORLD == (SHDIR == 2), "world-frame means take the direction from the camera centre, pre-transformed ones from the mean or the origin");
        float v[3];
        {
          const float xw[3] = {x0, x1, x2};
          sh_dir_vec<SHDIR>(ps, xw, p, v);
        }
        const float pinv = 1.f / sqrtf(v[0] * v[0] + v[1] * v[1] + v[2] * v[2]);
        const float ux = v[0] * pinv, uy = v[1] * pinv, uz = v[2] * pinv;
        sh_basis(in.sh_deg, ux, uy, uz, shb);
        float gbx[16], gby[16], gbz[16];
        sh_basis_grad(in.sh_deg, ux, uy, uz, gbx, gby, gbz);
        const int nb = (in.sh_deg + 1) * (in.sh_deg + 1);
        shg[0] = (cl_bits & 1) ? 0.f : dc0; shg[1] = (cl_bits & 2) ? 0.f : dc1; shg[2] = (cl_bits & 4) ? 0.f : dc2;
        const float* rest = in.f_rest + (size_t)idx * (size_t)in.n_rest * 3;
        float ddx = 0.f, ddy = 0.f, ddz = 0.f;
#pragma unroll
        for (int k = 1; k < 16; k++)
          if (k < nb) {
            const float tk = rest[(k - 1) * 3] * shg[0] + rest[(k - 1) * 3 + 1] * shg[1] + rest[(k - 1) * 3 + 2] * shg[2];
            ddx += gbx[k] * tk; ddy += gby[k] * tk; ddz += gbz[k] * tk;
          }
        const float dot = ux * ddx + uy * ddy + uz * ddz;
        if constexpr (SHDIR == 0) {
          dm[0] += (ddx - ux * dot) * pinv; dm[1] += (ddy - uy * dot) * pinv; dm[2] += (ddz - uz * dot) * pinv;
        } else {
          shw[0] = (ddx - ux * dot) * pinv; shw[1] = (ddy - uy * dot) * pinv; shw[2] = (ddz - uz * dot) * pinv;
        }
      }
      cg[0] = dm[0] * x0; cg[1] = dm[0] * x1; cg[2] = dm[0] * x2;
      cg[3] = dm[1] * x0; cg[4] = dm[1] * x1; cg[5] = dm[1] * x2;
      cg[6] = dm[2] * x0; cg[7] = dm[2] * x1; cg[8] = dm[2] * x2;
      cg[9] = dm[0]; cg[10] = dm[1]; cg[11] = dm[2];
      if (world) {
#pragma unroll
        for (int k = 0; k < 3; k++)
#pragma unroll
          for (int i = 0; i < 3; i++) cg[k * 3 + i] += dRc[k][i];
        cg[2] += dz_tot * x0; cg[5] += dz_tot * x1; cg[8] += dz_tot * x2;
      }
      if constexpr (SH && SHDIR == 2) {
#pragma unroll
        for (int i = 0; i < 3; i++) {
#pragma unroll
          for (int j = 0; j < 3; j++) cg[i * 3 + j] += ps.t[i] * shw[j];
          cg[9 + i] += ps.R[i][0] * shw[0] + ps.R[i][1] * shw[1] + ps.R[i][2] * shw[2];
        }
      }
      if (out.d_xyz || ma.on) {
#pragma unroll
        for (int j = 0; j < 3; j++) dxyz[j] = ps.R[0][j] * dm[0] + ps.R[1][j] * dm[1] + ps.R[2][j] * dm[2] + (world ? dz_tot * ps.R[j][2] : 0.f);
        if constexpr (SH && SHDIR != 0) {
#pragma unroll
          for (int j = 0; j < 3; j++) dxyz[j] += shw[j];
        }
        const uint32_t cl = cl_bits;
        dfd[0] = (cl & 1) ? 0.f : SH_C0F * dc0;
        dfd[1] = (cl & 2) ? 0.f : SH_C0F * dc1;
        dfd[2] = (cl & 4) ? 0.f : SH_C0F * dc2;
        const float o = 1.f / (1.f + expf(-op_raw));
        dlogit = M0 * (1.f - o);
        float dM[3][3], dR[3][3], ds[3];
#pragma unroll
        for (int i = 0; i < 3; i++)
#pragma unroll
          for (int k = 0; k < 3; k++) dM[i][k] = 2.f * (dS[i][0] * R[0][k] + dS[i][1] * R[1][k] + dS[i][2] * R[2][k]) * sm[k];
#pragma unroll
        for (int k = 0; k < 3; k++) {
          ds[k] = cam.scale_modifier * (dM[0][k] * R[0][k] + dM[1][k] * R[1][k] + dM[2][k] * R[2][k]);
#pragma unroll
          for (int i = 0; i < 3; i++) dR[i][k] = dM[i][k] * sm[k];
        }
        const float inv_mod = 1.f / cam.scale_modifier;
        if (in.isotropic) {
          dls[0] = (ds[0] * sm[0] + ds[1] * sm[1] + ds[2] * sm[2]) * inv_mod;
        } else {
          dls[0] = ds[0] * sm[0] * inv_mod; dls[1] = ds[1] * sm[1] * inv_mod; dls[2] = ds[2] * sm[2] * inv_mod;
        }
        dR_to_dq_raw(qn, qinv, dR, dqr);
      }
      if (out.max_radii2D) {
        out.max_radii2D[idx] = fmaxf(out.max_radii2D[idx], (float)rad);
        out.grad_accum[idx] += gnorm;
        out.denom[idx] += 1.f;
      }
    }
    if (out.d_xyz) {
      out.d_xyz[(size_t)idx * 3] = dxyz[0]; out.d_xyz[(size_t)idx * 3 + 1] = dxyz[1]; out.d_xyz[(size_t)idx * 3 + 2] = dxyz[2];
      out.d_f_dc[(size_t)idx * 3] = dfd[0]; out.d_f_dc[(size_t)idx * 3 + 1] = dfd[1]; out.d_f_dc[(size_t)idx * 3 + 2] = dfd[2];
      out.d_opacity[idx] = dlogit;
      out.d_scaling[(size_t)idx * 3] = dls[0]; out.d_scaling[(size_t)idx * 3 + 1] = dls[1]; out.d_scaling[(size_t)idx * 3 + 2] = dls[2];
      out.d_rotation[(size_t)idx * 4] = dqr[0]; out.d_rotation[(size_t)idx * 4 + 1] = dqr[1];
      out.d_rotation[(size_t)idx * 4 + 2] = dqr[2]; out.d_rotation[(size_t)idx * 4 + 3] = dqr[3];
      if constexpr (SH) {
        if (out.d_f_rest) {
          float* o = out.d_f_rest + (size_t)idx * (size_t)in.n_rest * 3;
          const int nb = (in.sh_deg + 1) * (in.sh_deg + 1);
#pragma unroll
          for (int k = 1; k < 16; k++)
            if (k - 1 < in.n_rest) {
              const float bk = k < nb ? shb[k] : 0.f;
              o[(k - 1) * 3] = bk * shg[0]; o[(k - 1) * 3 + 1] = bk * shg[1]; o[(k - 1) * 3 + 2] = bk * shg[2];
            }
        }
      }
    }
    if (ma.on) {
      const float keepg = (ma.opt_mask && ma.opt_mask[idx] == 0) ? 0.f : 1.f;
      const float gr14[14] = {keepg * dxyz[0], keepg * dxyz[1], keepg * dxyz[2], keepg * dfd[0], keepg * dfd[1], keepg * dfd[2], keepg * dlogit,
                              keepg * dls[0], keepg * dls[1], keepg * dls[2], keepg * dqr[0], keepg * dqr[1], keepg * dqr[2], keepg * dqr[3]};
      if (!skip) {
#pragma unroll
      for (int gq = 0; gq < 5; gq++)
#pragma unroll
        for (int c = 0; c < AG_N[gq]; c++) {
          const int q = AG_OFF[gq] + c;
          const size_t off = (size_t)idx * AG_N[gq] + c;
          const AdamElem r = adam_elem(ap[q], am[q], av[q], gr14[q], ma.omb1, ma.beta2, ma.omb2, ma.bc2s, ma.eps, ma.step_size[gq]);
          ma.m[gq][off] = r.m; ma.v[gq][off] = r.v;
          ap[q] = r.p;
          ma.p[gq][off] = ap[q];
        }
      if constexpr (SH) {
        if (ma.rp) {
          const int nb = (in.sh_deg + 1) * (in.sh_deg + 1);
          const size_t base = (size_t)idx * (size_t)in.n_rest * 3;
#pragma unroll
          for (int k = 1; k < 16; k++)
            if (k - 1 < in.n_rest) {
              const float bk = k < nb ? keepg * shb[k] : 0.f;
#pragma unroll
              for (int ch = 0; ch < 3; ch++) {
                const size_t off = base + (size_t)(k - 1) * 3 + ch;
                const float gr = bk * shg[ch];
                const float m0 = ma.rm[off], v0 = ma.rv[off];
                AdamElem r;
                adam_moments(m0, v0, gr, ma.omb1, ma.beta2, ma.omb2, r);
                ma.rm[off] = r.m; ma.rv[off] = r.v;
                ma.rp[off] = adam_param(ma.rp[off], r, ma.bc2s, ma.eps, ma.rest_step_size);
              }
            }
        }
      }
      }
      if (stepped) {
#pragma unroll
        for (int k = 0; k < 3; k++) { stepped->x[k] = ap[k]; stepped->fd[k] = ap[3 + k]; stepped->ls[k] = ap[7 + k]; }
        stepped->op = ap[6];
#pragma unroll
        for (int k = 0; k < 4; k++) stepped->q[k] = ap[10 + k];
      }
    }
  }
  if (posepartial) {
    __shared__ float red[SLAM_BWD_FB / 64][NPOSE];
    const int lane = threadIdx.x & 63, wv = threadIdx.x >> 6;
#pragma unroll
    for (int k = 0; k < NPOSE; k++) {
      float v = wave_sum_to_lane63(cg[k]);
      if (lane == 63) red[wv][k] = v;
    }
    __syncthreads();
    if (threadIdx.x < NPOSE) {
      const int k = threadIdx.x;
      float t = red[0][k];
#pragma unroll
      for (int w = 1; w < SLAM_BWD_FB / 64; w++) t += red[w][k];
      posepartial[(size_t)blockIdx.x * 32 + k] = t;
    }
  }
}

static_assert(SLAM_BWD_FB == FB, "the fused backward + projection kernel uses one lane per Gaussian in both halves");
template <bool WORLD>
__global__ void __launch_bounds__(FB)
slam_bwd_project_kernel(CamDev cam, int P, SlamIn in, int32_t* __restrict__ radii, GeomView g, ImageView iv, BinView b, uint32_t N_cap,
                        const float* __restrict__ dsub, SlamGrads out, MapAdam ma, const float* __restrict__ next_pose, uint32_t cap,
                        uint32_t rec_cap, int slot_bits) {
  extern __shared__ uint32_t hist[];
  const int idx = slam_bin_prologue(cam, iv, cap, hist);
  RawGaussian rg = {{0.f, 0.f, 0.f}, {1.f, 0.f, 0.f, 0.f}, {0.f, 0.f, 0.f}, {0.f, 0.f, 0.f}, 0.f};
  slam_bwd_body<false, true, WORLD>(cam, P, in, radii, g, N_cap, dsub, nullptr, out, ma, &rg, &iv.hdr->overflow_seen);
  const Projected pr = slam_project_vals(cam, idx < P, idx, next_pose, in.isotropic != 0, rg, radii, g, WORLD);
  slam_bin_pairs(cam, P, idx, pr, g, iv, b, cap, rec_cap, slot_bits, hist);
}

void launch_slam_bwd_project(const CamDev& cam, int P, const SlamIn& in, int32_t* radii, GeomView g, ImageView iv, BinView b, size_t N_cap,
                             BwdView bw, const SlamGrads& out, const MapAdam& ma, const float* next_pose, uint32_t bin_cap, uint32_t rec_cap,
                             int slot_bits, hipStream_t s) {
  if (P <= 0) return;
  const uint32_t ncap = (uint32_t)(N_cap > 0xffffffffull ? 0xffffffffull : N_cap);
  const int T = cam.gx * cam.gy;
  hipLaunchKernelGGL(in.world ? slam_bwd_project_kernel<true> : slam_bwd_project_kernel<false>, dim3((P + FB - 1) / FB), dim3(FB), (size_t)T * 4, s, cam, P, in,
                     radii, g, iv, b, ncap, bw.dsub, out, ma, next_pose, bin_cap, rec_cap, slot_bits);
}

template <bool WORLD, bool SH = false, int SHDIR = 0>
__global__ void __launch_bounds__(FB)
slam_adam_project_kernel(CamDev cam, int P, SlamIn in, int32_t* __restrict__ radii, GeomView g, ImageView iv, BinView b, SlamGrads gr, MapAdam ma,
                         const float* __restrict__ next_pose, uint32_t cap, uint32_t rec_cap, int slot_bits) {
  static_assert(!SH || WORLD == (SHDIR == 2), "world-frame means take the direction from the camera centre, pre-transformed ones from the mean or the origin");
  extern __shared__ uint32_t hist[];
  const int idx = slam_bin_prologue(cam, iv, cap, hist);
  RawGaussian rg = {{0.f, 0.f, 0.f}, {1.f, 0.f, 0.f, 0.f}, {0.f, 0.f, 0.f}, {0.f, 0.f, 0.f}, 0.f};
  float rs[SH ? 45 : 1];
  if (idx < P) {
    constexpr int AG_OFF[5] = {0, 3, 6, 7, 10}, AG_N[5] = {3, 3, 1, 3, 4};
    const float* gsrc[5] = {gr.d_xyz, gr.d_f_dc, gr.d_opacity, gr.d_scaling, gr.d_rotation};
    float ap[14], am[14], av[14], g14[14];
#pragma unroll
    for (int gq = 0; gq < 5; gq++)
#pragma unroll
      for (int c = 0; c < AG_N[gq]; c++) {
        const size_t off = (size_t)idx * AG_N[gq] + c;
        ap[AG_OFF[gq] + c] = ma.p[gq][off]; am[AG_OFF[gq] + c] = ma.m[gq][off]; av[AG_OFF[gq] + c] = ma.v[gq][off];
        g14[AG_OFF[gq] + c] = gsrc[gq][off];
      }
    const float keepg = (ma.opt_mask && ma.opt_mask[idx] == 0) ? 0.f : 1.f;
#pragma unroll
    for (int gq = 0; gq < 5; gq++)
#pragma unroll
      for (int c = 0; c < AG_N[gq]; c++) {
        const int q = AG_OFF[gq] + c;
        const size_t off = (size_t)idx * AG_N[gq] + c;
        const float grd = keepg * g14[q];
        AdamElem r;
        adam_moments(am[q], av[q], grd, ma.omb1, ma.beta2, ma.omb2, r);
        ma.m[gq][off] = r.m; ma.v[gq][off] = r.v;
        ap[q] = adam_param(ap[q], r, ma.bc2s, ma.eps, ma.step_size[gq]);
        ma.p[gq][off] = ap[q];
      }
    if constexpr (SH) {
      const int nb = (in.sh_deg + 1) * (in.sh_deg + 1);
      const size_t base = (size_t)idx * (size_t)in.n_rest * 3;
#pragma unroll
      for (int k = 1; k < 16; k++)
        if (k - 1 < in.n_rest) {
#pragma unroll
          for (int ch = 0; ch < 3; ch++) {
            const size_t off = base + (size_t)(k - 1) * 3 + ch;
            const float grd = k < nb ? keepg * gr.d_f_rest[off] : 0.f;
            const float m0 = ma.rm[off], v0 = ma.rv[off];
            AdamElem r;
            adam_moments(m0, v0, grd, ma.omb1, ma.beta2, ma.omb2, r);
            ma.rm[off] = r.m; ma.rv[off] = r.v;
            const float pn = adam_param(ma.rp[off], r, ma.bc2s, ma.eps, ma.rest_step_size);
            ma.rp[off] = pn;
            rs[(k - 1) * 3 + ch] = pn;
          }
        }
    }
#pragma unroll
    for (int k = 0; k < 3; k++) { rg.x[k] = ap[k]; rg.fd[k] = ap[3 + k]; rg.ls[k] = ap[7 + k]; }
    rg.op = ap[6];
#pragma unroll
    for (int k = 0; k < 4; k++) rg.q[k] = ap[10 + k];
  }
  if constexpr (SH) {
    const Projected pr = slam_project_vals<true, SHDIR>(cam, idx < P, idx, next_pose, in.isotropic != 0, rg, radii, g, WORLD, false, rs, in.sh_deg);
    slam_bin_pairs(cam, P, idx, pr, g, iv, b, cap, rec_cap, slot_bits, hist);
  } else {
    const Projected pr = slam_project_vals(cam, idx < P, idx, next_pose, in.isotropic != 0, rg, radii, g, WORLD);
    slam_bin_pairs(cam, P, idx, pr, g, iv, b, cap, rec_cap, slot_bits, hist);
  }
}

void launch_slam_adam_project(const CamDev& cam, int P, const SlamIn& in, int32_t* radii, GeomView g, ImageView iv, BinView b, const SlamGrads& gr,
                              const MapAdam& ma, const float* next_pose, uint32_t bin_cap, uint32_t rec_cap, int slot_bits, hipStream_t s) {
  if (P <= 0) return;
  const int T = cam.gx * cam.gy;
  auto k = in.sh_deg <= 0 ? (in.world ? slam_adam_project_kernel<true> : slam_adam_project_kernel<false>)
         : in.sh_dir == 2 ? slam_adam_project_kernel<true, true, 2> : in.sh_dir == 1 ? slam_adam_project_kernel<false, true, 1> : slam_adam_project_kernel<false, true, 0>;
  hipLaunchKernelGGL(k, dim3((P + FB - 1) / FB), dim3(FB), (size_t)T * 4, s, cam, P, in, radii, g, iv, b, gr, ma, next_pose, bin_cap, rec_cap, slot_bits);
}

__device__ __forceinline__ double pow_int(double b, int t) {
  double r = 1.0;
  for (; t > 0; t >>= 1) { if (t & 1) r *= b; b *= b; }
  return r;
}

template <int NG>
__device__ __forceinline__ void pose_finish_body(const float* __restrict__ posepartial, int nrows, const float* __restrict__ pose_in,
                                                 float* __restrict__ dpose, const PoseAdam& ad, const PoseLossScale& pls, float* __restrict__ ad_loss4,
                                                 const uint32_t* __restrict__ ovf) {
  static_assert(NG % 8 == 0, "row groups are folded eight at a time");
  __shared__ double part[NG][16];
  __shared__ double part8[NG / 8][16];
  __shared__ double tot[16];
  const int k = threadIdx.x;
  float pin[4] = {1.f, 0.f, 0.f, 0.f}, pcur[7], am[7], av[7], prior[7], ptr_in[3] = {0.f, 0.f, 0.f};
#pragma unroll
  for (int i = 0; i < 7; i++) { pcur[i] = 0.f; am[i] = 0.f; av[i] = 0.f; prior[i] = 0.f; }
  int step0 = 0;
  uint32_t ovf_word = 0u;
  if (k == 0) {
    if (ovf) ovf_word = *ovf;
#pragma unroll
    for (int i = 0; i < 4; i++) pin[i] = pose_in[i];
    if (ad.prior) {
#pragma unroll
      for (int i = 0; i < 7; i++) prior[i] = ad.prior[i];
#pragma unroll
      for (int i = 0; i < 3; i++) ptr_in[i] = pose_in[4 + i];
    }
    if (ad.pose) {
#pragma unroll
      for (int i = 0; i < 7; i++) { pcur[i] = ad.pose[i]; am[i] = ad.m[i]; av[i] = ad.v[i]; }
      step0 = *ad.step;
    }
  }
  {
    const int col = k & 15, grp = k >> 4;
    double a0 = 0.0, a1 = 0.0;
    if (col < NPOSE) {
      int r = grp;
      for (; r + 7 * NG < nrows; r += 8 * NG) {
        float v[8];
#pragma unroll
        for (int u = 0; u < 8; u++) v[u] = *(posepartial + (size_t)(r + u * NG) * 32 + col);
#pragma unroll
        for (int u = 0; u < 8; u += 2) { a0 += (double)v[u]; a1 += (double)v[u + 1]; }
      }
      {
        float v[8];
#pragma unroll
        for (int u = 0; u < 8; u++) v[u] = (r + u * NG < nrows) ? *(posepartial + (size_t)(r + u * NG) * 32 + col) : 0.f;
#pragma unroll
        for (int u = 0; u < 8; u += 2) { a0 += (double)v[u]; a1 += (double)v[u + 1]; }
      }
    } else if (pls.rows) {
      const double* lr = pls.rows + ((col - NPOSE) & 1);
      double b0 = 0.0, b1 = 0.0, b2 = 0.0, b3 = 0.0;
      int r = grp + NG * ((col - NPOSE) >> 1);
      for (; r + 6 * NG < pls.nrows; r += 8 * NG) {
        b0 += lr[(size_t)r * 12]; b1 += lr[(size_t)(r + 2 * NG) * 12]; b2 += lr[(size_t)(r + 4 * NG) * 12]; b3 += lr[(size_t)(r + 6 * NG) * 12];
      }
      for (; r < pls.nrows; r += 2 * NG) b0 += lr[(size_t)r * 12];
      a0 = (b0 + b1) + (b2 + b3);
    }
    part[grp][col] = a0 + a1;
  }
  __syncthreads();
  if ((k >> 4) < NG / 8) {
    double acc = 0.0;
#pragma unroll
    for (int gq = 0; gq < 8; gq++) acc += part[(k >> 4) * 8 + gq][k & 15];
    part8[k >> 4][k & 15] = acc;
  }
  __syncthreads();
  if (k < 16) {
    double acc = 0.0;
#pragma unroll
    for (int gq = 0; gq < NG / 8; gq++) acc += part8[gq][k];
    tot[k] = acc;
  }
  __syncthreads();
  if (k == 0) {
    if (pls.rows) {
      tot[NPOSE] += tot[NPOSE + 2]; tot[NPOSE + 1] += tot[NPOSE + 3];
      const double npx = tot[NPOSE + 1];
      const double sc = npx > 0.0 ? 1.0 / npx : 0.0;
      for (int i = 0; i < NPOSE; i++) tot[i] *= sc;
      if (pls.loss4) {
        const double l1 = npx > 0.0 ? tot[NPOSE] / (3.0 * npx) : 0.0;
        pls.loss4[0] = (float)(pls.w_l1 * l1); pls.loss4[1] = (float)l1; pls.loss4[2] = 0.f; pls.loss4[3] = 0.f;
      }
    }
    const float w0 = pin[0], x0 = pin[1], y0 = pin[2], z0 = pin[3];
    const float n = sqrtf(w0 * w0 + x0 * x0 + y0 * y0 + z0 * z0), inv = 1.f / n;
    float dR[3][3];
    for (int i = 0; i < 3; i++)
      for (int j = 0; j < 3; j++) dR[i][j] = (float)tot[i * 3 + j];
    const float qn[4] = {w0 * inv, x0 * inv, y0 * inv, z0 * inv};
    float grad[7];
    dR_to_dq_raw(qn, inv, dR, grad);
    for (int i = 0; i < 3; i++) grad[4 + i] = (float)tot[9 + i];
    if (ad.prior) {
      const float w2 = prior[0], x2 = -prior[1], y2 = -prior[2], z2 = -prior[3];
      const float d0 = w0 * w2 - x0 * x2 - y0 * y2 - z0 * z2, d1 = w0 * x2 + x0 * w2 + y0 * z2 - z0 * y2;
      const float d2 = w0 * y2 - x0 * z2 + y0 * w2 + z0 * x2, d3 = w0 * z2 + x0 * y2 - y0 * x2 + z0 * w2;
      const float dn = fmaxf(sqrtf(d0 * d0 + d1 * d1 + d2 * d2 + d3 * d3), 1e-12f), idn = 1.f / dn;
      const float u0 = d0 * idn, u1 = d1 * idn, u2 = d2 * idn, u3 = d3 * idn;
      const float s2 = 1.f - u0 * u0;
      float t_l = 0.f;
#pragma unroll
      for (int i = 0; i < 3; i++) { const float e = ptr_in[i] - prior[4 + i]; t_l += e * e; grad[4 + i] += ad.prior_w_t * 2.f * e; }
      const float ang = 2.f * acosf(fminf(fabsf(u0), 1.f));
      if (s2 > 0.f) {
        const float coef = ad.prior_w_q * -2.f * (u0 < 0.f ? -1.f : 1.f) / sqrtf(s2);
        const float g0 = coef * (1.f - u0 * u0) * idn, g1 = coef * (-u0 * u1) * idn, g2 = coef * (-u0 * u2) * idn, g3 = coef * (-u0 * u3) * idn;
        grad[0] += g0 * w2 + g1 * x2 + g2 * y2 + g3 * z2;
        grad[1] += -g0 * x2 + g1 * w2 - g2 * z2 + g3 * y2;
        grad[2] += -g0 * y2 + g1 * z2 + g2 * w2 - g3 * x2;
        grad[3] += -g0 * z2 - g1 * y2 + g2 * x2 + g3 * w2;
      }
      float* l4 = pls.loss4 ? pls.loss4 : ad_loss4;
      if (l4) l4[0] += ad.prior_w_t * t_l + ad.prior_w_q * ang;
    }
    float* const l4_total = pls.loss4 ? pls.loss4 : ad_loss4;
    if (dpose) for (int i = 0; i < 7; i++) dpose[i] = grad[i];
    if (ad.pose && ovf_word == 0u) {
      const int t = step0 + 1;
      *ad.step = t;
      const double bc1 = 1.0 - pow_int(ad.beta1, t);
      const float bc2s = (float)sqrt(1.0 - pow_int(ad.beta2, t));
      const float omb1 = (float)(1.0 - ad.beta1), b2 = (float)ad.beta2, omb2 = (float)(1.0 - ad.beta2);
      const float ss_q = (float)(ad.lr_q / bc1), ss_t = (float)(ad.lr_t / bc1);
      for (int i = 0; i < 7; i++) {
        const AdamElem r = adam_elem(pcur[i], am[i], av[i], grad[i], omb1, b2, omb2, bc2s, ad.eps, i < 4 ? ss_q : ss_t);
        ad.m[i] = r.m; ad.v[i] = r.v;
        pcur[i] = r.p;
        ad.pose[i] = pcur[i];
      }
      if (ad.best && l4_total) {
        const float lt = l4_total[0];
        if (lt < ad.best[0]) {
          ad.best[0] = lt;
          for (int i = 0; i < 7; i++) ad.best[1 + i] = pcur[i];
        }
      }
    }
  }
}

__global__ void __launch_bounds__(1024) slam_pose_finish_kernel(const float* __restrict__ posepartial, int nrows, const float* __restrict__ pose_in,
                                        float* __restrict__ dpose, PoseAdam ad, PoseLossScale pls, float* __restrict__ ad_loss4,
                                        const uint32_t* __restrict__ ovf) {
  pose_finish_body<64>(posepartial, nrows, pose_in, dpose, ad, pls, ad_loss4, ovf);
}

template <bool TRACK, bool DIRECT, bool WORLD, bool SH = false, int SHDIR = 0>
__global__ void __launch_bounds__(SLAM_BWD_FB)
slam_preprocess_bwd_kernel(CamDev cam, int P, SlamIn in, const int32_t* __restrict__ radii, GeomView g, BinView bn, uint32_t N_cap,
                           const float* __restrict__ dsub, float* __restrict__ posepartial, SlamGrads out, MapAdam ma,
                           const uint32_t* __restrict__ ovf) {
  slam_bwd_body<TRACK, DIRECT, WORLD, SH, SHDIR>(cam, P, in, radii, g, N_cap, dsub, posepartial, out, ma, nullptr, ovf);
}

void launch_slam_pose_finish(const float* rows, int nrows, const float* pose_in, float* dpose, const PoseAdam& ad, hipStream_t s,
                             const PoseLossScale* pls, float* loss4, const uint32_t* ovf) {
  const PoseLossScale none = {nullptr, 0, 0.f, nullptr};
  hipLaunchKernelGGL(slam_pose_finish_kernel, dim3(1), dim3(1024), 0, s, rows, nrows, pose_in, dpose, ad, pls ? *pls : none, loss4, ovf);
}

template <bool DIRECT>
static auto pick_slam_preprocess_bwd(const SlamIn& in, bool map) -> decltype(&slam_preprocess_bwd_kernel<false, DIRECT, false>) {
  if (in.sh_deg > 0)
    return in.sh_dir == 2 ? slam_preprocess_bwd_kernel<false, DIRECT, true, true, 2>
         : in.sh_dir == 1 ? slam_preprocess_bwd_kernel<false, DIRECT, false, true, 1> : slam_preprocess_bwd_kernel<false, DIRECT, false, true, 0>;
  if (in.world) return map ? slam_preprocess_bwd_kernel<false, DIRECT, true> : slam_preprocess_bwd_kernel<true, DIRECT, true>;
  return map ? slam_preprocess_bwd_kernel<false, DIRECT, false> : slam_preprocess_bwd_kernel<true, DIRECT, false>;
}

void launch_slam_preprocess_bwd(const CamDev& cam, int P, const SlamIn& in, const int32_t* radii, GeomView g, BinView b, size_t N_cap,
                                BwdView bw, const SlamGrads& out, float* dpose, const PoseAdam& ad, const MapAdam& ma, hipStream_t s,
                                const PoseLossScale* pls, float* loss4, bool direct, const uint32_t* ovf) {
  const uint32_t ncap = (uint32_t)(N_cap > 0xffffffffull ? 0xffffffffull : N_cap);
  const bool want_pose = dpose != nullptr || ad.pose != nullptr;
  float* partial = want_pose ? bw.campartial : nullptr;
  if (P > 0) {
    const bool map = out.d_xyz || ma.on;
    auto kern = direct ? pick_slam_preprocess_bwd<true>(in, map) : pick_slam_preprocess_bwd<false>(in, map);
    hipLaunchKernelGGL(kern, dim3((P + SLAM_BWD_FB - 1) / SLAM_BWD_FB), dim3(SLAM_BWD_FB), 0, s, cam, P, in, radii, g, b, ncap, bw.dsub, partial, out, ma, ovf);
  }
  if (want_pose) launch_slam_pose_finish(bw.campartial, P > 0 ? (P + SLAM_BWD_FB - 1) / SLAM_BWD_FB : 0, in.pose, dpose, ad, s, pls, loss4, ovf);
}

__global__ void __launch_bounds__(256) fused_adam_kernel(AdamArgs a) {
  const unsigned long long tid = (unsigned long long)blockIdx.x * 256 + threadIdx.x;
  const unsigned long long stride = (unsigned long long)gridDim.x * 256;
  for (int gi = 0; gi < a.ngroups; gi++) {
    const AdamGroup G = a.grp[gi];
    const float step = G.step_size;
    const bool vec = ((G.n & 3ull) == 0) && ((((uintptr_t)G.p | (uintptr_t)G.g | (uintptr_t)G.m | (uintptr_t)G.v) & 15) == 0);
    if (vec) {
      const unsigned long long n4 = G.n >> 2;
      float4* p4 = (float4*)G.p; const float4* g4 = (const float4*)G.g; float4* m4 = (float4*)G.m; float4* v4 = (float4*)G.v;
      for (unsigned long long i = tid; i < n4; i += stride) {
        float4 pr = p4[i], gr = g4[i], mi = m4[i], vi = v4[i];
        float* pp = (float*)&pr; const float* gg = (const float*)&gr; float* mm = (float*)&mi; float* vv = (float*)&vi;
#pragma unroll
        for (int c = 0; c < 4; c++) {
          const AdamElem r = adam_elem(pp[c], mm[c], vv[c], gg[c], a.omb1, a.beta2, a.omb2, a.bc2s, a.eps, step);
          mm[c] = r.m; vv[c] = r.v; pp[c] = r.p;
        }
        p4[i] = pr; m4[i] = mi; v4[i] = vi;
      }
    } else {
      for (unsigned long long i = tid; i < G.n; i += stride) {
        const float gr = G.g[i];
        const AdamElem r = adam_elem(G.p[i], G.m[i], G.v[i], gr, a.omb1, a.beta2, a.omb2, a.bc2s, a.eps, step);
        G.m[i] = r.m; G.v[i] = r.v; G.p[i] = r.p;
      }
    }
  }
}
void launch_fused_adam(const AdamArgs& a, hipStream_t s) {
  unsigned long long tot = 0;
  for (int i = 0; i < a.ngroups; i++) tot = tot > a.grp[i].n ? tot : a.grp[i].n;
  if (!tot) return;
  int blocks = (int)((tot / 4 + 255) / 256) + 1;
  if (blocks > 2048) blocks = 2048;
  hipLaunchKernelGGL(fused_adam_kernel, dim3(blocks), dim3(256), 0, s, a);
}
```

mm3dgs_slam_amd/csrc/fused_api.h:

```cpp
#pragma once
#include "mm3dgs_common.h"

struct SlamIn {
  const float* pose; const float* xyz; const float* f_dc; const float* opacity; const float* scaling; const float* rotation;
  int isotropic;
  int world;
  const float* f_rest; int sh_deg; int n_rest;
  int sh_dir;
};
struct SlamGrads {
  float* d_xyz; float* d_f_dc; float* d_opacity; float* d_scaling; float* d_rotation;
  float* max_radii2D; float* grad_accum; float* denom;
  float* d_f_rest;
};
struct MapAdam { float* p[5]; float* m[5]; float* v[5]; float step_size[5]; float omb1, beta2, omb2, eps, bc2s; int on; const uint8_t* opt_mask;
                 float* rp; float* rm; float* rv; float rest_step_size; };
struct PoseAdam { float* pose; float* m; float* v; int* step; double lr_q, lr_t, beta1, beta2; float eps; const float* prior; float prior_w_t, prior_w_q; float* best; };
struct AdamGroup { float* p; const float* g; float* m; float* v; unsigned long long n; float step_size; };
struct AdamArgs { AdamGroup grp[8]; int ngroups; float omb1, beta2, omb2, eps, bc2s; };
struct LossCfg {
  int H, W;
  float w_l1, w_ssim, w_pearson;
  int l1_mask, pearson_mask, pearson_invert;
  float sil_thr;
  float window[11];
  float w_depth;
  int depth_mask;
  int l1_sum;
};

struct TrackLoss {
  LossCfg cfg;
  const float* gt;
  const float* ref;
  const float* out;
  const float* dmaps;
  double* partial;
  const double* sums;
  float* loss4;
  int defer_scale;
};
struct PoseLossScale { const double* rows; int nrows; float w_l1; float* loss4; };
void launch_loss_finish(const LossCfg& cfg, double* sums, const double* partial, hipStream_t s, float* loss4 = nullptr);

void launch_slam_preprocess_fwd(const CamDev& cam, int P, const SlamIn& in, int32_t* radii, GeomView g, ImageView iv, hipStream_t s,
                                uint32_t* seen_only = nullptr, bool visibility_only = false, bool want_poserec = false);
void launch_slam_pose_finish(const float* rows, int nrows, const float* pose_in, float* dpose, const PoseAdam& ad, hipStream_t s,
                             const PoseLossScale* pls, float* loss4, const uint32_t* ovf);
void launch_slam_preprocess_bwd(const CamDev& cam, int P, const SlamIn& in, const int32_t* radii, GeomView g, BinView b, size_t N_cap,
                                BwdView bw, const SlamGrads& out, float* dpose, const PoseAdam& ad, const MapAdam& ma, hipStream_t s,
                                const PoseLossScale* pls = nullptr, float* loss4 = nullptr, bool direct = false, const uint32_t* overflow_flag = nullptr);
void launch_composite_bwd_slam(const CamDev& cam, bool tracking, GeomView g, ImageView iv, BinView b, size_t N_cap, const float* dL,
                               float* dsub, hipStream_t s, const TrackLoss* tl = nullptr, int dl_planes = 6, bool pose_chain = false);
void launch_sort_composite_fwd6(const CamDev& cam, GeomView g, ImageView iv, BinView b, size_t N_cap, float* out, int clean, hipStream_t s,
                                const TrackLoss* tl = nullptr, int direct_blocks = 0, uint32_t direct_cap = 0, int slot_bits = DIRECT_SLOT_BITS_MAX);
void launch_sort_composite_fwd_bwd_track(const CamDev& cam, GeomView g, ImageView iv, BinView b, size_t N_cap, float* out, int clean,
                                         hipStream_t s, const TrackLoss& tl, int direct_blocks, float* dsub, uint32_t direct_cap = 0, int slot_bits = DIRECT_SLOT_BITS_MAX,
                                         bool pose_chain = false);
void launch_slam_bwd_project(const CamDev& cam, int P, const SlamIn& in, int32_t* radii, GeomView g, ImageView iv, BinView b, size_t N_cap,
                             BwdView bw, const SlamGrads& out, const MapAdam& ma, const float* next_pose, uint32_t bin_cap, uint32_t rec_cap,
                             int slot_bits, hipStream_t s);
void launch_slam_project_bin(const CamDev& cam, int P, const SlamIn& in, int32_t* radii, GeomView g, ImageView iv, BinView b, uint32_t bin_cap,
                             uint32_t rec_cap, int slot_bits, hipStream_t s, bool want_poserec = false);
void launch_slam_adam_project(const CamDev& cam, int P, const SlamIn& in, int32_t* radii, GeomView g, ImageView iv, BinView b, const SlamGrads& gr,
                              const MapAdam& ma, const float* next_pose, uint32_t bin_cap, uint32_t rec_cap, int slot_bits, hipStream_t s);
void launch_fused_adam(const AdamArgs& a, hipStream_t s);
void launch_loss(const LossCfg& cfg, const float* out, const float* gt, const float* ref, float* dmaps, double* sums, double* partial,
                 float* dL, float* loss, hipStream_t s);
void launch_loss_after_forward_rows(const LossCfg& cfg, const float* out, const float* gt, const float* ref, float* dmaps, double* sums,
                                    double* partial, float* dL, hipStream_t s);

struct CompactTable { const float* src[32]; float* dst[32]; int width[32]; int n_arrays; };
struct SeedOut { float* xyz; float* f_dc; float* f_rest; float* opacity; float* scaling; float* rotation; float* rgb; int n_rest; };
void launch_prune_mask(int P, const float* opacity, const float* scaling, const float* max_radii2D, float min_opacity, float max_scale,
                       float max_screen_size, int use_screen, uint8_t* keep, uint32_t* n_pruned, hipStream_t s);
void launch_compact_plan(int n, const uint8_t* keep, uint32_t* block_pre, uint32_t* n_keep, hipStream_t s);
void launch_compact_rows(int n, const uint8_t* keep, const uint32_t* block_pre, const CompactTable& t, hipStream_t s);
struct DensifyTable {
  const float* src[7]; float* dst[7]; const float* m_src[7]; float* m_dst[7]; const float* v_src[7]; float* v_dst[7]; int width[7];
  float* grad_accum; float* denom; float* max_radii2D; int32_t* parent;
};
void launch_densify_plan(int P, const float* grad_accum, const float* denom, const float* scaling, float max_grad, float max_clone_scale,
                         uint8_t* cls, uint32_t* block_counts, uint32_t* counts, hipStream_t s);
void launch_densify_rows(int P, const uint8_t* cls, const uint32_t* block_pre, uint32_t n_keep, uint32_t n_clone, uint32_t n_split, int N,
                         uint32_t seed, float shrink, const DensifyTable& t, hipStream_t s);
void launch_seed_gaussians(int H, int W, const float* color, const float* depth, const uint8_t* keep, const uint32_t* block_pre,
                           const float* pose, float fx, float fy, float cx, float cy, uint32_t row0, const SeedOut& o, hipStream_t s);

void launch_covisibility_ratio(int H, int W, const float* depth, const float* sil, const float* kf_pose, const float* cur_pose, float fx, float fy,
                               float cx, float cy, uint32_t* counts, hipStream_t s);
void launch_propagate_const_vel(const float* pm1, const float* pm2, float* out, hipStream_t s);
void launch_propagate_imu(const float* pm1, const float* pm2, const float* imu6, int n, const float* c2i, double dt_cam, double dt_imu,
                          double gx, double gy, double gz, float* out, hipStream_t s);
```

Baseline: 31.85.

## Fold pose-finish Adam step into next iteration's project-bin kernel

In the tracking loop, the single-block pose-finish kernel (row reduction plus pose Adam update) is no longer launched between iterations. Every block of the next iteration's project-and-bin kernel now redundantly reduces the per-tile pose partial rows and applies the Adam step itself, then projects Gaussians with the updated pose held in shared memory. Block 0 writes the pose, Adam state and best-pose values into double-buffered device slots, and overflow is tracked through pending flags. This removes one serialized one-block launch per tracking iteration. In exchange every projection block repeats the reduction work, and the pose, overflow and best-loss bookkeeping becomes considerably more complex.

```diff
diff --git a/mm3dgs_slam_amd/csrc/api.hip b/mm3dgs_slam_amd/csrc/api.hip
--- a/mm3dgs_slam_amd/csrc/api.hip
+++ b/mm3dgs_slam_amd/csrc/api.hip
@@ -198,7 +198,7 @@
 static void warn_env_once() {
   static const bool done = [] {
     static const char* const names[] = {"MM3DGS_NO_DIRECT_BINS", "MM3DGS_NO_FUSED_SORT", "MM3DGS_NO_FUSED_SCAN", "MM3DGS_NO_FUSED_TRACK", "MM3DGS_NO_FOLDED_LOSS",
-                                        "MM3DGS_NO_FORWARD_ROWS", "MM3DGS_NO_FUSED_PROJECT", "MM3DGS_NO_TILE_ORDER", "MM3DGS_NO_POSE_CHAIN", "MM3DGS_TILEMAP",
+                                        "MM3DGS_NO_FORWARD_ROWS", "MM3DGS_NO_FUSED_PROJECT", "MM3DGS_NO_TILE_ORDER", "MM3DGS_NO_POSE_CHAIN", "MM3DGS_NO_FOLDED_FINISH", "MM3DGS_TILEMAP",
                                         "MM3DGS_DIRECT_MAX_TILES", "MM3DGS_STATS", "MM3DGS_SLAM_LDS_PAD", "MM3DGS_FWD_LDS_PAD", "MM3DGS_BWD_LDS_PAD"};
     for (const char* n : names) {
       const char* v = getenv(n);
@@ -269,9 +269,25 @@
   launch_tile_order(cd.gx * cd.gy, cd.H, cd.W, image_view(image_state, cd.H, cd.W), (hipStream_t)stream);
 }
 
+static int pose_adam_dev(const Mm3dgsPoseAdam* pose_adam, PoseAdam& pa) {
+  pa = PoseAdam{};
+  if (pose_adam && pose_adam->pose) {
+    if (!pose_adam->m || !pose_adam->v || !pose_adam->step) return fail(-2, "pose Adam state missing");
+    pa.pose = pose_adam->pose; pa.m = pose_adam->m; pa.v = pose_adam->v; pa.step = pose_adam->step;
+    pa.lr_q = pose_adam->lr_q; pa.lr_t = pose_adam->lr_t; pa.beta1 = pose_adam->beta1; pa.beta2 = pose_adam->beta2; pa.eps = (float)pose_adam->eps;
+    if (pose_adam->prior_pose && (pose_adam->prior_w_t != 0.f || pose_adam->prior_w_q != 0.f)) {
+      pa.prior = pose_adam->prior_pose; pa.prior_w_t = pose_adam->prior_w_t; pa.prior_w_q = pose_adam->prior_w_q;
+    }
+    pa.best = pose_adam->best;
+  }
+  return 0;
+}
+struct FoldedFinish { int it; PoseAdam pa; PoseLossScale pls; PoseFold fold; PoseSeed seed; };
+
 static int slam_forward_impl(const Mm3dgsCamera* cam, int P, const Mm3dgsSlamInputs* in, float* out_color, int32_t* radii,
                              void* geom_state, void* image_state, void* binning_state, size_t N_capacity, int flags, void* stream,
-                             const TrackLoss* tl, float* track_dsub = nullptr, bool projected = false, bool pose_chain = false) {
+                             const TrackLoss* tl, float* track_dsub = nullptr, bool projected = false, bool pose_chain = false,
+                             const FoldedFinish* ff = nullptr) {
   int rc = check_slam(cam, P, in);
   if (rc) return rc;
   if (!out_color || !geom_state || !image_state || !binning_state || (P > 0 && !radii)) return fail(-1, "NULL buffer");
@@ -292,7 +308,11 @@
   const DirectBins db = slam_direct_bins(flags, cd, P, N_capacity);
   cd.trec_cap = db.on ? db.trec_cap : 0u;
   if (db.on) {
-    if (!projected) { ProfScope ps(MM3DGS_PROF_PREPROCESS_FWD, s); launch_slam_project_bin(cd, P, slam_in(in), radii, g, iv, b, db.bin_cap, db.rec_cap, db.slot_bits, s, pose_chain); }
+    if (ff && !projected && ff->it > 0) {
+      ProfScope ps(MM3DGS_PROF_PREPROCESS_FWD, s);
+      launch_slam_finish_project_bin(cd, P, slam_in(in), radii, g, iv, b, db.bin_cap, db.rec_cap, db.slot_bits, s, track_dsub, ff->pa, ff->pls, ff->fold);
+    } else
+    if (!projected) { ProfScope ps(MM3DGS_PROF_PREPROCESS_FWD, s); launch_slam_project_bin(cd, P, slam_in(in), radii, g, iv, b, db.bin_cap, db.rec_cap, db.slot_bits, s, pose_chain, ff ? &ff->seed : nullptr); }
     { ProfScope ps(track_dsub ? MM3DGS_PROF_TRACK_FWD_BWD : MM3DGS_PROF_COMPOSITE_FWD, s);
       if (track_dsub) launch_sort_composite_fwd_bwd_track(cd, g, iv, b, N_capacity, out_color, 1, s, *tl, db.nblocks, track_dsub, db.bin_cap, db.slot_bits, pose_chain);
       else launch_sort_composite_fwd6(cd, g, iv, b, N_capacity, out_color, 1, s, tl, db.nblocks, db.bin_cap, db.slot_bits); }
@@ -349,7 +369,7 @@
                               const float* dL_dout, void* backward_scratch, const Mm3dgsSlamGrads* grads, float* dL_dpose,
                               const Mm3dgsPoseAdam* pose_adam, const Mm3dgsMapAdam* map_adam, int flags, void* stream, const TrackLoss* tl,
                               float* prior_loss4 = nullptr, int dl_planes = 6, bool compositor_done = false, const float* fuse_next_pose = nullptr,
-                              bool* fused_out = nullptr, bool pose_chain = false) {
+                              bool* fused_out = nullptr, bool pose_chain = false, const PoseFold* last_fold = nullptr) {
   PoseLossScale pls = {nullptr, 0, 0.f, nullptr};
   if (tl && tl->defer_scale) { pls.rows = tl->partial; pls.nrows = ((tl->cfg.W + 15) / 16) * ((tl->cfg.H + 15) / 16); pls.w_l1 = tl->cfg.w_l1; pls.loss4 = tl->loss4; }
   int rc = check_slam(cam, P, in);
@@ -376,16 +396,8 @@
     sg.d_f_rest = (all && in->sh_degree > 0) ? grads->d_f_rest : nullptr;
     if (all && in->sh_degree > 0 && !grads->d_f_rest) return fail(-2, "sh_degree > 0: the gradient outputs need d_f_rest too");
   }
-  PoseAdam pa = {};
-  if (pose_adam && pose_adam->pose) {
-    if (!pose_adam->m || !pose_adam->v || !pose_adam->step) return fail(-2, "pose Adam state missing");
-    pa.pose = pose_adam->pose; pa.m = pose_adam->m; pa.v = pose_adam->v; pa.step = pose_adam->step;
-    pa.lr_q = pose_adam->lr_q; pa.lr_t = pose_adam->lr_t; pa.beta1 = pose_adam->beta1; pa.beta2 = pose_adam->beta2; pa.eps = (float)pose_adam->eps;
-    if (pose_adam->prior_pose && (pose_adam->prior_w_t != 0.f || pose_adam->prior_w_q != 0.f)) {
-      pa.prior = pose_adam->prior_pose; pa.prior_w_t = pose_adam->prior_w_t; pa.prior_w_q = pose_adam->prior_w_q;
-    }
-    pa.best = pose_adam->best;
-  }
+  PoseAdam pa;
+  if (int rc2 = pose_adam_dev(pose_adam, pa)) return rc2;
   MapAdam ma;
   memset(&ma, 0, sizeof(ma));
   if (map_adam)
@@ -400,7 +412,7 @@
     launch_composite_bwd_slam(cd, tracking, g, iv, b, N_capacity, dL_dout, bw.dsub, s, tl, dl_planes, pose_chain); }
   if (pose_chain) {
     ProfScope ps(MM3DGS_PROF_PREPROCESS_BWD, s);
-    launch_slam_pose_finish(bw.dsub, cd.gx * cd.gy, in->pose, dL_dpose, pa, s, pls.rows ? &pls : nullptr, prior_loss4, &iv.hdr->overflow);
+    launch_slam_pose_finish(bw.dsub, cd.gx * cd.gy, in->pose, dL_dpose, pa, s, pls.rows ? &pls : nullptr, prior_loss4, &iv.hdr->overflow, last_fold);
     return check_launch("slam_backward");
   }
   const bool fuse = fuse_next_pose && !tracking && ma.on && db_bwd.on && !dL_dpose && !pa.pose && !sg.d_xyz && !sh;
@@ -487,9 +499,32 @@
   }
   const bool pose_chain = !in->world_means && !sh && backward_scratch && !env_flag("MM3DGS_NO_POSE_CHAIN", 0) &&
                           bwd_bytes_impl(P, N_capacity) >= (size_t)tiles_x(cam->image_width) * tiles_y(cam->image_height) * 32 * sizeof(float);
+  FoldedFinish ff = {};
+  bool fold_finish = false;
+  if (pose_chain && fuse_track && n_iter > 1 && P > 0 && in->pose == pose_adam->pose && !env_flag("MM3DGS_NO_FOLDED_FINISH", 0)) {
+    const CamDev cd = cam_dev(cam);
+    const BwdView bw = bwd_view(backward_scratch, P, N_capacity);
+    const size_t row_bytes = (size_t)cd.gx * cd.gy * 32 * sizeof(float);
+    if (slam_direct_bins(fwd_flags, cd, P, N_capacity).on && (size_t)((char*)bw.campartial - (char*)bw.dsub) >= row_bytes) {
+      if (int rc = pose_adam_dev(pose_adam, ff.pa)) return rc;
+      ff.pls.rows = tl.partial; ff.pls.nrows = (int)loss_rows(tl.cfg.H, tl.cfg.W); ff.pls.w_l1 = tl.cfg.w_l1; ff.pls.loss4 = tl.loss4;
+      ff.seed.slot = bw.campartial + POSE_SLOT_F;
+      ff.seed.pend = (uint32_t*)(bw.campartial + 2 * POSE_SLOT_F);
+      ff.seed.pose = ff.pa.pose; ff.seed.m = ff.pa.m; ff.seed.v = ff.pa.v; ff.seed.step = ff.pa.step; ff.seed.best = ff.pa.best;
+      ff.fold.ovf_live = &image_view(image_state, cd.H, cd.W).hdr->overflow;
+      fold_finish = true;
+    }
+  }
   if (n_iter > 0) slam_refresh_tile_order(cam, image_state, fwd_flags, stream);
   for (int it = 0; it < n_iter; it++) {
-    int rc = slam_forward_impl(cam, P, in, out_color, radii, geom_state, image_state, binning_state, N_capacity, fwd_flags, stream, fold ? &tl : nullptr, track_dsub, false, pose_chain);
+    if (fold_finish) {
+      float* slots = ff.seed.slot - POSE_SLOT_F;
+      ff.it = it;
+      ff.fold.src = slots + (it & 1) * POSE_SLOT_F; ff.fold.dst = slots + ((it + 1) & 1) * POSE_SLOT_F;
+      ff.fold.pend = ff.seed.pend + ((it + 1) & 1); ff.fold.pend_out = ff.seed.pend + (it & 1);
+    }
+    int rc = slam_forward_impl(cam, P, in, out_color, radii, geom_state, image_state, binning_state, N_capacity, fwd_flags, stream, fold ? &tl : nullptr, track_dsub, false, pose_chain,
+                               fold_finish ? &ff : nullptr);
     if (rc) return rc;
     if (fold) {
       if (!tl.defer_scale) {
@@ -500,8 +535,12 @@
       rc = mm3dgs_loss(loss_cfg, out_color, gt_color, ref, loss_work, dL_dout, loss4, stream);
       if (rc) return rc;
     }
+    if (fold_finish && it + 1 < n_iter) continue;
+    PoseFold last = {};
+    if (fold_finish) { last.pend = ff.seed.pend + (it & 1); last.ovf_live = ff.fold.ovf_live; }
     rc = slam_backward_impl(cam, P, in, radii, geom_state, image_state, binning_state, N_capacity, dL_dout, backward_scratch, &none,
-                            nullptr, pose_adam, nullptr, fwd_flags, stream, fold ? &tl : nullptr, loss4, 6, fuse_track, nullptr, nullptr, pose_chain);
+                            nullptr, pose_adam, nullptr, fwd_flags, stream, fold ? &tl : nullptr, loss4, 6, fuse_track, nullptr, nullptr, pose_chain,
+                            fold_finish ? &last : nullptr);
     if (rc) return rc;
   }
   return 0;
diff --git a/mm3dgs_slam_amd/csrc/fused.hip b/mm3dgs_slam_amd/csrc/fused.hip
--- a/mm3dgs_slam_amd/csrc/fused.hip
+++ b/mm3dgs_slam_amd/csrc/fused.hip
@@ -195,20 +195,25 @@
   return o;
 }
 
+__device__ __forceinline__ RawGaussian slam_load_raw(const SlamIn& in, bool live, int idx) {
+  RawGaussian rg = {{0.f, 0.f, 0.f}, {1.f, 0.f, 0.f, 0.f}, {0.f, 0.f, 0.f}, {0.f, 0.f, 0.f}, 0.f};
+  if (live) {
+#pragma unroll
+    for (int k = 0; k < 3; k++) rg.x[k] = in.xyz[(size_t)idx * 3 + k];
+#pragma unroll
+    for (int k = 0; k < 4; k++) rg.q[k] = in.rotation[(size_t)idx * 4 + k];
+#pragma unroll
+    for (int k = 0; k < 3; k++) { rg.ls[k] = in.scaling[(size_t)idx * 3 + k]; rg.fd[k] = in.f_dc[(size_t)idx * 3 + k]; }
+    rg.op = in.opacity[idx];
+  }
+  return rg;
+}
+
 template <bool SH = false, int SHDIR = 0>
 __device__ __forceinline__ Projected slam_project_one(const CamDev& cam, int P, int idx, const SlamIn& in, int32_t* __restrict__ radii,
                                                       const GeomView& g, bool want_poserec = false) {
   const bool live = idx < P;
-  RawGaussian rg = {{0.f, 0.f, 0.f}, {1.f, 0.f, 0.f, 0.f}, {0.f, 0.f, 0.f}, {0.f, 0.f, 0.f}, 0.f};
-  if (live) {
-#pragma unroll
-    for (int k = 0; k < 3; k++) rg.x[k] = in.xyz[(size_t)idx * 3 + k];
-#pragma unroll
-    for (int k = 0; k < 4; k++) rg.q[k] = in.rotation[(size_t)idx * 4 + k];
-#pragma unroll
-    for (int k = 0; k < 3; k++) { rg.ls[k] = in.scaling[(size_t)idx * 3 + k]; rg.fd[k] = in.f_dc[(size_t)idx * 3 + k]; }
-    rg.op = in.opacity[idx];
-  }
+  const RawGaussian rg = slam_load_raw(in, live, idx);
   return slam_project_vals<SH, SHDIR>(cam, live, idx, in.pose, in.isotropic != 0, rg, radii, g, in.world != 0, want_poserec,
                                SH ? in.f_rest + (size_t)(live ? idx : 0) * (size_t)in.n_rest * 3 : nullptr, in.sh_deg);
 }
@@ -297,7 +302,8 @@
 }
 
 __device__ __forceinline__ void slam_bin_pairs(const CamDev& cam, int P, int idx, const Projected& pr, const GeomView& g, const ImageView& iv,
-                                               const BinView& b, uint32_t cap, uint32_t rec_cap, int slot_bits, uint32_t* hist) {
+                                               const BinView& b, uint32_t cap, uint32_t rec_cap, int slot_bits, uint32_t* hist,
+                                               uint32_t* ovf_out = nullptr) {
   const int T = cam.gx * cam.gy;
   const int tid = threadIdx.x, lane = tid & 63, wvi = tid >> 6;
   const bool live = idx < P;
@@ -321,7 +327,7 @@
     c.trec0 = plocal + (uint32_t)c.area <= cam.trec_cap ? (uint32_t)blockIdx.x * cam.trec_cap + plocal : 0xffffffffu;
     if (tid == FB - 1) {
       g.block_tiles[blockIdx.x] = pre2 + x2;
-      if (pre2 + x2 > cam.trec_cap) iv.hdr->overflow = 1u;
+      if (pre2 + x2 > cam.trec_cap) *(ovf_out ? ovf_out : &iv.hdr->overflow) = 1u;
     }
   }
   constexpr int OWN = 4;
@@ -400,19 +406,31 @@
 template <bool SH, int SHDIR = 0>
 __global__ void __launch_bounds__(FB)
 slam_project_bin_kernel(CamDev cam, int P, SlamIn in, int32_t* __restrict__ radii, GeomView g, ImageView iv, BinView b, uint32_t cap,
-                        uint32_t rec_cap, int slot_bits, int want_poserec) {
+                        uint32_t rec_cap, int slot_bits, int want_poserec, PoseSeed seed) {
   extern __shared__ uint32_t hist[];
   const int idx = slam_bin_prologue(cam, iv, cap, hist);
+  if (seed.slot && blockIdx.x == 0 && threadIdx.x < POSE_SLOT_F) {
+    const int t = threadIdx.x;
+    float w = 0.f;
+    if (t < 7) w = seed.pose[t];
+    else if (t < 14) w = seed.m[t - 7];
+    else if (t < 21) w = seed.v[t - 14];
+    else if (t == 21) w = __int_as_float(*seed.step);
+    else if (t < 30 && seed.best) w = seed.best[t - 22];
+    seed.slot[t] = w;
+    if (t < 2) seed.pend[t] = 0u;
+  }
   const Projected pr = slam_project_one<SH, SHDIR>(cam, P, idx, in, radii, g, want_poserec != 0);
   slam_bin_pairs(cam, P, idx, pr, g, iv, b, cap, rec_cap, slot_bits, hist);
 }
 
 void launch_slam_project_bin(const CamDev& cam, int P, const SlamIn& in, int32_t* radii, GeomView g, ImageView iv, BinView b, uint32_t bin_cap,
-                             uint32_t rec_cap, int slot_bits, hipStream_t s, bool want_poserec) {
+                             uint32_t rec_cap, int slot_bits, hipStream_t s, bool want_poserec, const PoseSeed* seed) {
   if (P <= 0) return;
   const int T = cam.gx * cam.gy;
+  const PoseSeed none = {};
   hipLaunchKernelGGL(SLAM_PICK_SH(slam_project_bin_kernel, in), dim3((P + FB - 1) / FB), dim3(FB), (size_t)T * 4, s, cam, P, in, radii, g, iv, b, bin_cap,
-                     rec_cap, slot_bits, want_poserec && in.sh_deg <= 0 ? 1 : 0);
+                     rec_cap, slot_bits, want_poserec && in.sh_deg <= 0 ? 1 : 0, seed ? *seed : none);
 }
 
 template <bool TRACK>
@@ -871,66 +889,108 @@
   return r;
 }
 
-template <int NG>
+template <int NG, int NT>
 __device__ __forceinline__ void pose_finish_body(const float* __restrict__ posepartial, int nrows, const float* __restrict__ pose_in,
                                                  float* __restrict__ dpose, const PoseAdam& ad, const PoseLossScale& pls, float* __restrict__ ad_loss4,
-                                                 const uint32_t* __restrict__ ovf) {
+                                                 const uint32_t* ovf, const PoseFold& fold, float* pose_out) {
   static_assert(NG % 8 == 0, "row groups are folded eight at a time");
+  static_assert((16 * NG) % NT == 0 && NT % 16 == 0 && NT / 16 >= NG / 8, "lanes = 16 columns x a divisor of the row groups, enough for the first fold");
+  constexpr int NPER = 16 * NG / NT;
+  constexpr int GSTEP = NT / 16;
   __shared__ double part[NG][16];
   __shared__ double part8[NG / 8][16];
   __shared__ double tot[16];
   const int k = threadIdx.x;
-  float pin[4] = {1.f, 0.f, 0.f, 0.f}, pcur[7], am[7], av[7], prior[7], ptr_in[3] = {0.f, 0.f, 0.f};
+  const bool writer = blockIdx.x == 0;
+  float pin[4] = {1.f, 0.f, 0.f, 0.f}, pcur[7], am[7], av[7], prior[7], ptr_in[3] = {0.f, 0.f, 0.f}, bst[8];
 #pragma unroll
   for (int i = 0; i < 7; i++) { pcur[i] = 0.f; am[i] = 0.f; av[i] = 0.f; prior[i] = 0.f; }
+#pragma unroll
+  for (int i = 0; i < 8; i++) bst[i] = 0.f;
   int step0 = 0;
-  uint32_t ovf_word = 0u;
+  uint32_t ovf_word = 0u, pend_word = 0u;
   if (k == 0) {
     if (ovf) ovf_word = *ovf;
-#pragma unroll
-    for (int i = 0; i < 4; i++) pin[i] = pose_in[i];
+    if (fold.pend) pend_word = *fold.pend;
+    const float* pq = fold.src ? fold.src : pose_in;
+#pragma unroll
+    for (int i = 0; i < 4; i++) pin[i] = pq[i];
     if (ad.prior) {
 #pragma unroll
       for (int i = 0; i < 7; i++) prior[i] = ad.prior[i];
 #pragma unroll
-      for (int i = 0; i < 3; i++) ptr_in[i] = pose_in[4 + i];
-    }
-    if (ad.pose) {
+      for (int i = 0; i < 3; i++) ptr_in[i] = pq[4 + i];
+    }
+    if (fold.src) {
+#pragma unroll
+      for (int i = 0; i < 7; i++) { pcur[i] = fold.src[i]; am[i] = fold.src[7 + i]; av[i] = fold.src[14 + i]; }
+      step0 = __float_as_int(fold.src[21]);
+      if (ad.best) {
+#pragma unroll
+        for (int i = 0; i < 8; i++) bst[i] = fold.src[22 + i];
+      }
+    } else if (ad.pose) {
 #pragma unroll
       for (int i = 0; i < 7; i++) { pcur[i] = ad.pose[i]; am[i] = ad.m[i]; av[i] = ad.v[i]; }
       step0 = *ad.step;
+      if (ad.best) bst[0] = ad.best[0];
     }
   }
   {
     const int col = k & 15, grp = k >> 4;
-    double a0 = 0.0, a1 = 0.0;
+    double a0[NPER], a1[NPER];
+#pragma unroll
+    for (int j = 0; j < NPER; j++) { a0[j] = 0.0; a1[j] = 0.0; }
     if (col < NPOSE) {
-      int r = grp;
-      for (; r + 7 * NG < nrows; r += 8 * NG) {
-        float v[8];
-#pragma unroll
-        for (int u = 0; u < 8; u++) v[u] = *(posepartial + (size_t)(r + u * NG) * 32 + col);
-#pragma unroll
-        for (int u = 0; u < 8; u += 2) { a0 += (double)v[u]; a1 += (double)v[u + 1]; }
-      }
-      {
-        float v[8];
-#pragma unroll
-        for (int u = 0; u < 8; u++) v[u] = (r + u * NG < nrows) ? *(posepartial + (size_t)(r + u * NG) * 32 + col) : 0.f;
-#pragma unroll
-        for (int u = 0; u < 8; u += 2) { a0 += (double)v[u]; a1 += (double)v[u + 1]; }
+      for (int base = 0; base < nrows; base += 8 * NG) {
+        float v[NPER][8];
+#pragma unroll
+        for (int j = 0; j < NPER; j++)
+#pragma unroll
+          for (int u = 0; u < 8; u++) {
+            const int r = base + grp + j * GSTEP + u * NG;
+            v[j][u] = r < nrows ? *(posepartial + (size_t)r * 32 + col) : 0.f;
+          }
+#pragma unroll
+        for (int j = 0; j < NPER; j++)
+#pragma unroll
+          for (int u = 0; u < 8; u += 2) { a0[j] += (double)v[j][u]; a1[j] += (double)v[j][u + 1]; }
       }
     } else if (pls.rows) {
       const double* lr = pls.rows + ((col - NPOSE) & 1);
-      double b0 = 0.0, b1 = 0.0, b2 = 0.0, b3 = 0.0;
-      int r = grp + NG * ((col - NPOSE) >> 1);
-      for (; r + 6 * NG < pls.nrows; r += 8 * NG) {
-        b0 += lr[(size_t)r * 12]; b1 += lr[(size_t)(r + 2 * NG) * 12]; b2 += lr[(size_t)(r + 4 * NG) * 12]; b3 += lr[(size_t)(r + 6 * NG) * 12];
-      }
-      for (; r < pls.nrows; r += 2 * NG) b0 += lr[(size_t)r * 12];
-      a0 = (b0 + b1) + (b2 + b3);
-    }
-    part[grp][col] = a0 + a1;
+      double b0[NPER], b1[NPER], b2[NPER], b3[NPER];
+      int r[NPER];
+#pragma unroll
+      for (int j = 0; j < NPER; j++) { b0[j] = 0.0; b1[j] = 0.0; b2[j] = 0.0; b3[j] = 0.0; r[j] = grp + j * GSTEP + NG * ((col - NPOSE) >> 1); }
+      for (;;) {
+        double w[NPER][4];
+        bool any = false;
+#pragma unroll
+        for (int j = 0; j < NPER; j++) {
+          const bool m = r[j] + 6 * NG < pls.nrows;
+          any = any || m;
+#pragma unroll
+          for (int q = 0; q < 4; q++) w[j][q] = m ? lr[(size_t)(r[j] + 2 * NG * q) * 12] : 0.0;
+          if (m) r[j] += 8 * NG;
+        }
+        if (!any) break;
+#pragma unroll
+        for (int j = 0; j < NPER; j++) { b0[j] += w[j][0]; b1[j] += w[j][1]; b2[j] += w[j][2]; b3[j] += w[j][3]; }
+      }
+      {
+        double w[NPER][3];
+#pragma unroll
+        for (int j = 0; j < NPER; j++)
+#pragma unroll
+          for (int q = 0; q < 3; q++) w[j][q] = r[j] + 2 * NG * q < pls.nrows ? lr[(size_t)(r[j] + 2 * NG * q) * 12] : 0.0;
+#pragma unroll
+        for (int j = 0; j < NPER; j++) { b0[j] += w[j][0]; b0[j] += w[j][1]; b0[j] += w[j][2]; }
+      }
+#pragma unroll
+      for (int j = 0; j < NPER; j++) a0[j] = (b0[j] + b1[j]) + (b2[j] + b3[j]);
+    }
+#pragma unroll
+    for (int j = 0; j < NPER; j++) part[grp + j * GSTEP][col] = a0[j] + a1[j];
   }
   __syncthreads();
   if ((k >> 4) < NG / 8) {
@@ -948,6 +1008,9 @@
   }
   __syncthreads();
   if (k == 0) {
+    float* const l4 = pls.loss4 ? pls.loss4 : ad_loss4;
+    float l0 = 0.f;
+    bool have_l0 = false;
     if (pls.rows) {
       tot[NPOSE] += tot[NPOSE + 2]; tot[NPOSE + 1] += tot[NPOSE + 3];
       const double npx = tot[NPOSE + 1];
@@ -955,7 +1018,8 @@
       for (int i = 0; i < NPOSE; i++) tot[i] *= sc;
       if (pls.loss4) {
         const double l1 = npx > 0.0 ? tot[NPOSE] / (3.0 * npx) : 0.0;
-        pls.loss4[0] = (float)(pls.w_l1 * l1); pls.loss4[1] = (float)l1; pls.loss4[2] = 0.f; pls.loss4[3] = 0.f;
+        l0 = (float)(pls.w_l1 * l1); have_l0 = true;
+        if (writer) { pls.loss4[0] = l0; pls.loss4[1] = (float)l1; pls.loss4[2] = 0.f; pls.loss4[3] = 0.f; }
       }
     }
     const float w0 = pin[0], x0 = pin[1], y0 = pin[2], z0 = pin[3];
@@ -986,39 +1050,79 @@
         grad[2] += -g0 * y2 + g1 * z2 + g2 * w2 - g3 * x2;
         grad[3] += -g0 * z2 - g1 * y2 + g2 * x2 + g3 * w2;
       }
-      float* l4 = pls.loss4 ? pls.loss4 : ad_loss4;
-      if (l4) l4[0] += ad.prior_w_t * t_l + ad.prior_w_q * ang;
-    }
-    float* const l4_total = pls.loss4 ? pls.loss4 : ad_loss4;
-    if (dpose) for (int i = 0; i < 7; i++) dpose[i] = grad[i];
-    if (ad.pose && ovf_word == 0u) {
+      if (l4) {
+        if (!have_l0) { l0 = l4[0]; have_l0 = true; }
+        l0 += ad.prior_w_t * t_l + ad.prior_w_q * ang;
+        if (writer) l4[0] = l0;
+      }
+    }
+    if (dpose && writer) for (int i = 0; i < 7; i++) dpose[i] = grad[i];
+    if (ad.pose && (ovf_word | pend_word) == 0u) {
       const int t = step0 + 1;
-      *ad.step = t;
+      step0 = t;
       const double bc1 = 1.0 - pow_int(ad.beta1, t);
       const float bc2s = (float)sqrt(1.0 - pow_int(ad.beta2, t));
       const float omb1 = (float)(1.0 - ad.beta1), b2 = (float)ad.beta2, omb2 = (float)(1.0 - ad.beta2);
       const float ss_q = (float)(ad.lr_q / bc1), ss_t = (float)(ad.lr_t / bc1);
       for (int i = 0; i < 7; i++) {
         const AdamElem r = adam_elem(pcur[i], am[i], av[i], grad[i], omb1, b2, omb2, bc2s, ad.eps, i < 4 ? ss_q : ss_t);
-        ad.m[i] = r.m; ad.v[i] = r.v;
-        pcur[i] = r.p;
-        ad.pose[i] = pcur[i];
-      }
-      if (ad.best && l4_total) {
-        const float lt = l4_total[0];
-        if (lt < ad.best[0]) {
-          ad.best[0] = lt;
-          for (int i = 0; i < 7; i++) ad.best[1 + i] = pcur[i];
-        }
-      }
+        am[i] = r.m; av[i] = r.v; pcur[i] = r.p;
+      }
+      bool better = false;
+      if (ad.best && l4) {
+        const float lt = have_l0 ? l0 : l4[0];
+        if (lt < bst[0]) {
+          better = true;
+          bst[0] = lt;
+          for (int i = 0; i < 7; i++) bst[1 + i] = pcur[i];
+        }
+      }
+      if (writer) {
+        *ad.step = t;
+        for (int i = 0; i < 7; i++) { ad.m[i] = am[i]; ad.v[i] = av[i]; ad.pose[i] = pcur[i]; }
+        if (better) for (int i = 0; i < 8; i++) ad.best[i] = bst[i];
+      }
+    }
+    if (pose_out) for (int i = 0; i < 7; i++) pose_out[i] = pcur[i];
+    if (writer) {
+      if (fold.dst) {
+        for (int i = 0; i < 7; i++) { fold.dst[i] = pcur[i]; fold.dst[7 + i] = am[i]; fold.dst[14 + i] = av[i]; }
+        fold.dst[21] = __int_as_float(step0);
+        for (int i = 0; i < 8; i++) fold.dst[22 + i] = bst[i];
+      }
+      if (pend_word) *fold.ovf_live = 1u;
     }
   }
 }
 
 __global__ void __launch_bounds__(1024) slam_pose_finish_kernel(const float* __restrict__ posepartial, int nrows, const float* __restrict__ pose_in,
                                         float* __restrict__ dpose, PoseAdam ad, PoseLossScale pls, float* __restrict__ ad_loss4,
-                                        const uint32_t* __restrict__ ovf) {
-  pose_finish_body<64>(posepartial, nrows, pose_in, dpose, ad, pls, ad_loss4, ovf);
+                                        const uint32_t* ovf, PoseFold fold) {
+  pose_finish_body<64, 1024>(posepartial, nrows, pose_in, dpose, ad, pls, ad_loss4, ovf, fold, nullptr);
+}
+
+__global__ void __launch_bounds__(FB)
+slam_finish_project_bin_kernel(CamDev cam, int P, SlamIn in, int32_t* __restrict__ radii, GeomView g, ImageView iv, BinView b, uint32_t cap,
+                               uint32_t rec_cap, int slot_bits, int want_poserec, const float* __restrict__ rows, int nrows, PoseAdam ad,
+                               PoseLossScale pls, PoseFold fold) {
+  extern __shared__ uint32_t hist[];
+  __shared__ float s_pose[8];
+  const int idx = slam_bin_prologue(cam, iv, cap, hist);
+  const bool live = idx < P;
+  const RawGaussian rg = slam_load_raw(in, live, idx);
+  pose_finish_body<64, FB>(rows, nrows, nullptr, nullptr, ad, pls, nullptr, &iv.hdr->overflow, fold, s_pose);
+  __syncthreads();
+  const Projected pr = slam_project_vals(cam, live, idx, s_pose, in.isotropic != 0, rg, radii, g, false, want_poserec != 0);
+  slam_bin_pairs(cam, P, idx, pr, g, iv, b, cap, rec_cap, slot_bits, hist, fold.pend_out);
+}
+
+void launch_slam_finish_project_bin(const CamDev& cam, int P, const SlamIn& in, int32_t* radii, GeomView g, ImageView iv, BinView b, uint32_t bin_cap,
+                                    uint32_t rec_cap, int slot_bits, hipStream_t s, const float* rows, const PoseAdam& ad, const PoseLossScale& pls,
+                                    const PoseFold& fold) {
+  if (P <= 0) return;
+  const int T = cam.gx * cam.gy;
+  hipLaunchKernelGGL(slam_finish_project_bin_kernel, dim3((P + FB - 1) / FB), dim3(FB), (size_t)T * 4, s, cam, P, in, radii, g, iv, b, bin_cap, rec_cap,
+                     slot_bits, 1, rows, T, ad, pls, fold);
 }
 
 template <bool TRACK, bool DIRECT, bool WORLD, bool SH = false, int SHDIR = 0>
@@ -1030,9 +1134,10 @@
 }
 
 void launch_slam_pose_finish(const float* rows, int nrows, const float* pose_in, float* dpose, const PoseAdam& ad, hipStream_t s,
-                             const PoseLossScale* pls, float* loss4, const uint32_t* ovf) {
+                             const PoseLossScale* pls, float* loss4, const uint32_t* ovf, const PoseFold* fold) {
   const PoseLossScale none = {nullptr, 0, 0.f, nullptr};
-  hipLaunchKernelGGL(slam_pose_finish_kernel, dim3(1), dim3(1024), 0, s, rows, nrows, pose_in, dpose, ad, pls ? *pls : none, loss4, ovf);
+  const PoseFold nofold = {};
+  hipLaunchKernelGGL(slam_pose_finish_kernel, dim3(1), dim3(1024), 0, s, rows, nrows, pose_in, dpose, ad, pls ? *pls : none, loss4, ovf, fold ? *fold : nofold);
 }
 
 template <bool DIRECT>
diff --git a/mm3dgs_slam_amd/csrc/fused_api.h b/mm3dgs_slam_amd/csrc/fused_api.h
--- a/mm3dgs_slam_amd/csrc/fused_api.h
+++ b/mm3dgs_slam_amd/csrc/fused_api.h
@@ -41,12 +41,21 @@
   int defer_scale;
 };
 struct PoseLossScale { const double* rows; int nrows; float w_l1; float* loss4; };
+#define POSE_SLOT_F 32
+struct PoseFold {
+  const float* src;
+  float* dst;
+  const uint32_t* pend;
+  uint32_t* pend_out;
+  uint32_t* ovf_live;
+};
+struct PoseSeed { float* slot; uint32_t* pend; const float* pose; const float* m; const float* v; const int* step; const float* best; };
 void launch_loss_finish(const LossCfg& cfg, double* sums, const double* partial, hipStream_t s, float* loss4 = nullptr);
 
 void launch_slam_preprocess_fwd(const CamDev& cam, int P, const SlamIn& in, int32_t* radii, GeomView g, ImageView iv, hipStream_t s,
                                 uint32_t* seen_only = nullptr, bool visibility_only = false, bool want_poserec = false);
 void launch_slam_pose_finish(const float* rows, int nrows, const float* pose_in, float* dpose, const PoseAdam& ad, hipStream_t s,
-                             const PoseLossScale* pls, float* loss4, const uint32_t* ovf);
+                             const PoseLossScale* pls, float* loss4, const uint32_t* ovf, const PoseFold* fold = nullptr);
 void launch_slam_preprocess_bwd(const CamDev& cam, int P, const SlamIn& in, const int32_t* radii, GeomView g, BinView b, size_t N_cap,
                                 BwdView bw, const SlamGrads& out, float* dpose, const PoseAdam& ad, const MapAdam& ma, hipStream_t s,
                                 const PoseLossScale* pls = nullptr, float* loss4 = nullptr, bool direct = false, const uint32_t* overflow_flag = nullptr);
@@ -61,7 +70,10 @@
                              BwdView bw, const SlamGrads& out, const MapAdam& ma, const float* next_pose, uint32_t bin_cap, uint32_t rec_cap,
                              int slot_bits, hipStream_t s);
 void launch_slam_project_bin(const CamDev& cam, int P, const SlamIn& in, int32_t* radii, GeomView g, ImageView iv, BinView b, uint32_t bin_cap,
-                             uint32_t rec_cap, int slot_bits, hipStream_t s, bool want_poserec = false);
+                             uint32_t rec_cap, int slot_bits, hipStream_t s, bool want_poserec = false, const PoseSeed* seed = nullptr);
+void launch_slam_finish_project_bin(const CamDev& cam, int P, const SlamIn& in, int32_t* radii, GeomView g, ImageView iv, BinView b, uint32_t bin_cap,
+                                    uint32_t rec_cap, int slot_bits, hipStream_t s, const float* rows, const PoseAdam& ad, const PoseLossScale& pls,
+                                    const PoseFold& fold);
 void launch_slam_adam_project(const CamDev& cam, int P, const SlamIn& in, int32_t* radii, GeomView g, ImageView iv, BinView b, const SlamGrads& gr,
                               const MapAdam& ma, const float* next_pose, uint32_t bin_cap, uint32_t rec_cap, int slot_bits, hipStream_t s);
 void launch_fused_adam(const AdamArgs& a, hipStream_t s);
```

Measured after the change: 30.37. 4.7% lower.
